# Huvinesh-Rajendran-12/keras-geometric

Measured on AMD Instinct MI355X. Metric: aggregated edges/sec + achieved HBM GB/s, GCNConv fwd, 1/2/4/8 MI355X, higher is better.
Workload: dtype fp32; 1 GPU; GCNConv fwd, R-MAT 10000000 nodes / 100000000 edges (+self loops), normalized, bias, F 128->128; nodes=10000000, edges=100000000, nodes_per_gpu=10000000, e_agg_per_gpu=110000000, max_in_degree=138539, mode=split-hub, fused aggregate->transform (W on bf16x3-split MFMA, f32-accurate), parallelism=single

## Files before the change

### include/kgx.h

```cpp
#ifndef KGX_H_
#define KGX_H_

#include <stddef.h>
#include <stdint.h>

#ifdef __cplusplus
extern "C" {
#endif

typedef void* kgx_stream_t;

enum kgx_status {
  KGX_OK = 0,
  KGX_ERR_ARG = 1,
  KGX_ERR_HIP = 2,
  KGX_ERR_INDEX = 3,
  KGX_ERR_UNSUPPORTED = 4
};

enum kgx_reduce { KGX_SUM = 0, KGX_MEAN = 1, KGX_MAX = 2, KGX_MIN = 3, KGX_STD = 4 };

enum kgx_epilogue { KGX_EPI_NONE = 0, KGX_EPI_BIAS = 1, KGX_EPI_GIN = 2, KGX_EPI_RAW = 3, KGX_EPI_ACCUM = 4 };

enum kgx_csr_flags {
  KGX_CSR_SELF_LOOPS = 1,
  KGX_CSR_SEGMENT_ONLY = 2,
  KGX_CSR_GCN_NORM = 4
};

int kgx_version(void);
const char* kgx_last_error(void);

int kgx_cu_split_layout_ok(int cus, int xccs, const char* arch);
int kgx_cu_split_supported(int device);
int kgx_cu_split_census(int per32, int64_t n_blocks, int32_t* head_ids, int32_t* tail_ids, int* n_cus,
                        kgx_stream_t stream);

int kgx_csr_workspace_bytes(int64_t E, int64_t n_dst, int flags, size_t* bytes);
int kgx_csr_build(const int32_t* src, const int32_t* dst, int64_t E,
                  int64_t n_src, int64_t n_dst, int flags,
                  int32_t* rowptr, int32_t* col, int32_t* eid, int32_t* deg,
                  float* dinv, float* w,
                  void* workspace, size_t workspace_bytes,
                  int64_t* info, kgx_stream_t stream);
int kgx_csr_build2(const int32_t* src, const int32_t* dst, int64_t E,
                   int64_t n_src, int64_t n_dst, int flags,
                   int32_t* rowptr, int32_t* col, int32_t* eid, int32_t* deg,
                   float* dinv, float* w, const float* dinv_table, int64_t table_len,
                   void* workspace, size_t workspace_bytes,
                   int64_t* info, kgx_stream_t stream);

int kgx_schedule_suffixes(const int32_t* items, int64_t n_items, int short_max, int tiny_max,
                          void* workspace, int64_t* out, kgx_stream_t stream);
int kgx_tiny_pack(const int32_t* items, int64_t start, int64_t n, const int32_t* col, const float* w,
                  int64_t n_col, int32_t* pack, float* tw, void* workspace, int64_t* out,
                  kgx_stream_t stream);

int kgx_gcn_dinv(const int32_t* deg, int64_t n, float* dinv, kgx_stream_t stream);
int kgx_gcn_dinv_table(const int32_t* deg, int64_t n, const float* table, int64_t table_len,
                       float* dinv, kgx_stream_t stream);
int kgx_gcn_edge_norm(const int32_t* rowptr, const int32_t* col, int64_t n_dst,
                      const float* dinv_dst, const float* dinv_src, float* w,
                      kgx_stream_t stream);

int kgx_schedule_workspace_bytes(int64_t n_dst, size_t* bytes);
int kgx_schedule_build(const int32_t* rowptr, int64_t n_dst, int32_t split_len,
                       int32_t* rows, int32_t* items, int64_t cap_items,
                       int32_t* split, void* workspace, size_t workspace_bytes,
                       int64_t* info, kgx_stream_t stream);

int kgx_spmm(int reduce, int epilogue,
             const int32_t* rowptr, const int32_t* rows, int64_t n_rows,
             const int32_t* items, int64_t n_items,
             const int32_t* split, int64_t n_split,
             const int32_t* idx, const float* w,
             const float* table, int64_t ld_table, int64_t F,
             float* out, int64_t ld_out,
             const float* bias, const float* xroot, int64_t ld_x, float gin_scale,
             const int32_t* drop_key, float drop_p, uint64_t drop_seed,
             float* partials, kgx_stream_t stream);
int kgx_spmm_ex(int reduce, int epilogue, const int32_t* rowptr, const int32_t* rows, int64_t n_rows,
                const int32_t* items, int64_t n_items, int64_t n_long_items, const int32_t* split,
                int64_t n_split, const int32_t* idx, const float* w, const float* table, int64_t ld_table,
                int64_t F, float* out, int64_t ld_out, const float* bias, const float* xroot, int64_t ld_x,
                float gin_scale, const int32_t* drop_key, float drop_p, uint64_t drop_seed, float* partials,
                kgx_stream_t stream);

int kgx_spmm_ex2(int reduce, int epilogue, const int32_t* rowptr, const int32_t* rows, int64_t n_rows,
                 const int32_t* items, int64_t n_items, int64_t n_long_items, const int32_t* split, int64_t n_split,
                 const int32_t* idx, const float* w, const float* table, int64_t ld_table, const float* table2,
                 int64_t n_table1, int64_t F, float* out, int64_t ld_out, const float* bias, const float* xroot,
                 int64_t ld_x, float gin_scale, const int32_t* drop_key, float drop_p, uint64_t drop_seed,
                 float* partials, int32_t* counters, kgx_stream_t stream);

int kgx_dropout_mask(uint64_t seed, float p, const int32_t* keys, int64_t n, int64_t F, float* out,
                     kgx_stream_t stream);

enum { KGX_FUSED_PRE_GIN = 1, KGX_FUSED_ACCUMULATE = 2, KGX_FUSED_SHARE_GPU = 4, KGX_FUSED_RELU = 8,
       KGX_FUSED_CU_SPLIT = 16 };
int kgx_spmm_gemm(int reduce, const int32_t* rowptr, const int32_t* rows, int64_t n_rows,
                  const int32_t* items, int64_t n_items, const int32_t* split, int64_t n_split,
                  const int32_t* idx, const float* w, const float* x, int64_t ld_x, int64_t F_in,
                  const float* W, int64_t F_out, const float* bias, int flags, float gin_scale,
                  float* out, int64_t ld_out, float* partials, float* agg_out, int64_t ld_agg,
                  kgx_stream_t stream);
enum { KGX_SHORT_ROW_MAX = 7 };
int kgx_spmm_gemm_ex(int reduce, const int32_t* rowptr, const int32_t* rows, int64_t n_rows,
                     const int32_t* items, int64_t n_items, int64_t n_long_items, const int32_t* split,
                     int64_t n_split, const int32_t* idx, const float* w, const float* x, int64_t ld_x,
                     int64_t F_in, const float* W, int64_t F_out, const float* bias, int flags,
                     float gin_scale, float* out, int64_t ld_out, float* partials, float* agg_out,
                     int64_t ld_agg, kgx_stream_t stream);

int kgx_spmm_gemm_ex2(int reduce, const int32_t* rowptr, const int32_t* rows, int64_t n_rows,
                      const int32_t* items, int64_t n_items, int64_t n_long_items, int64_t n_short_end,
                      const int32_t* tiny_pack, const float* tiny_w, int64_t n_tiny_deg2,
                      const int32_t* split, int64_t n_split,
                      const int32_t* idx, const float* w, const float* x, int64_t ld_x, int64_t F_in,
                      const float* W, int64_t F_out, const float* bias, int flags, float gin_scale, float* out,
                      int64_t ld_out, float* partials, float* agg_out, int64_t ld_agg, kgx_stream_t stream);

int kgx_spmm_gemm_ex3(int reduce, const int32_t* rowptr, const int32_t* rows, int64_t n_rows,
                      const int32_t* items, int64_t n_items, int64_t n_long_items, int64_t n_short_end,
                      const int32_t* tiny_pack, const float* tiny_w, int64_t n_tiny_deg2,
                      const int32_t* split, int64_t n_split, const int32_t* idx, const float* w,
                      const float* x, int64_t ld_x, const float* x2, int64_t n_x1, int64_t F_in,
                      const float* W, int64_t F_out, const float* bias, int flags, float gin_scale, float* out,
                      int64_t ld_out, float* partials, float* agg_out, int64_t ld_agg, kgx_stream_t stream);

int kgx_spmm_gemm_f256(int reduce, const int32_t* rowptr, const int32_t* rows, int64_t n_rows,
                       const int32_t* items, int64_t n_items, int64_t n_long_items, int64_t n_short_end,
                       const int32_t* tiny_pack, const float* tiny_w, const int32_t* split, int64_t n_split,
                       const int32_t* idx, const float* w, const float* x, int64_t ld_x, int64_t F_in,
                       const float* W, int64_t F_out, const float* bias, int flags, float gin_scale,
                       float* out, int64_t ld_out, float* partials, float* agg_out, int64_t ld_agg,
                       kgx_stream_t stream);

int kgx_spmm_gemm_f256_ex(int reduce, const int32_t* rowptr, const int32_t* rows, int64_t n_rows,
                          const int32_t* items, int64_t n_items, int64_t n_long_items, int64_t n_short_end,
                          const int32_t* tiny_pack, const float* tiny_w, const int32_t* split, int64_t n_split,
                          const int32_t* idx, const float* w, const float* x, int64_t ld_x, const float* x2,
                          int64_t n_x1, int64_t F_in, const float* W, int64_t F_out, const float* bias, int flags,
                          float gin_scale, float* out, int64_t ld_out, float* partials, float* agg_out,
                          int64_t ld_agg, kgx_stream_t stream);

int kgx_gemm_tn_workspace_bytes(int64_t N, int64_t K, int64_t M, size_t* bytes);
int kgx_gemm_tn(int64_t N, const float* P, int64_t ldp, int64_t K, const float* D, int64_t ldd, int64_t M,
                float* dW, int64_t ld_dw, float* db, void* workspace, size_t workspace_bytes,
                kgx_stream_t stream);

int kgx_spmm_max_backward(int reduce, int raw, const int32_t* rowptr, int64_t n_rows, const int32_t* idx,
                          const float* table, int64_t ld_table, int64_t F,
                          const float* grad_out, int64_t ld_grad_out,
                          float* grad_table, int64_t ld_grad_table, kgx_stream_t stream);

int kgx_gatv2(const int32_t* rowptr, const int32_t* rows, int64_t n_rows,
              const int32_t* items, int64_t n_items,
              const int32_t* split, int64_t n_split,
              const int32_t* col, const float* h_src, const float* h_dst, int64_t ld_h,
              const float* att, int heads, int channels, float negative_slope,
              float* out, int64_t ld_out, const float* bias,
              float* partials, float* stats,
              const int32_t* drop_key, float drop_p, uint64_t drop_seed, kgx_stream_t stream);

int kgx_gatv2_backward(const int32_t* rowptr, const int32_t* rows, int64_t n_rows,
                       const int32_t* items, int64_t n_items, const int32_t* split, int64_t n_split,
                       const int32_t* col, const float* h_src, const float* h_dst, int64_t ld_h,
                       const float* att, int heads, int channels, float negative_slope,
                       const float* out, int64_t ld_out, const float* bias, const float* stats,
                       const float* grad_out, int64_t ld_grad,
                       const int32_t* t_rowptr, const int32_t* t_rows, int64_t n_src,
                       const int32_t* t_items, int64_t t_n_items, const int32_t* t_split, int64_t t_n_split,
                       const int32_t* t_col, const int32_t* t_slot,
                       float* grad_h_src, float* grad_h_dst, int64_t ld_grad_h, float* grad_att,
                       float* alpha_ws, float* ds_ws, float* partials,
                       const int32_t* drop_key, float drop_p, uint64_t drop_seed, kgx_stream_t stream);

enum { KGX_POOL_SCORE_TANH = 1 };
enum { KGX_POOL_MAX_F = 256 };
int kgx_softmax_pool(const int32_t* rowptr, const int32_t* rows, int64_t n_seg,
                     const int32_t* items, int64_t n_items, const int32_t* split, int64_t n_split,
                     const int32_t* idx, const float* x, int64_t ld_x, int64_t F,
                     const float* s, const float* score_u, const float* score_c, int flags, float* s_out,
                     float* out, int64_t ld_out, float* stats, float* partials, kgx_stream_t stream);

int kgx_softmax_pool_backward(int64_t N, int64_t n_seg, const int32_t* seg,
                              const float* x, int64_t ld_x, int64_t F,
                              const float* s, const float* stats, const float* out, int64_t ld_out,
                              const float* grad_out, int64_t ld_grad,
                              float* grad_x, int64_t ld_grad_x, float* grad_s, kgx_stream_t stream);

enum { KGX_DENSE_RELU = 1, KGX_DENSE_ACCUMULATE = 2 };
enum { KGX_DENSE_MAX_K = 256, KGX_DENSE_MAX_N = 256 };
int kgx_dense(int64_t M, const float* x0, int64_t ld_x0, int64_t K0, const float* W0,
              const float* x1, int64_t ld_x1, int64_t K1, const float* W1, int64_t N,
              const float* bias, int flags, float* out, int64_t ld_out, kgx_stream_t stream);

int kgx_gather_rows(const float* table, int64_t ld_table, const int32_t* rows,
                    int64_t n, int64_t F, float* out, int64_t ld_out,
                    kgx_stream_t stream);
int kgx_scatter_f32(const float* in, const int32_t* perm, int64_t n, float* out,
                    kgx_stream_t stream);

int kgx_rmat_edges(uint64_t seed, int scale, int64_t n_nodes,
                   uint32_t a24, uint32_t b24, uint32_t c24,
                   int64_t e_begin, int64_t e_count,
                   int32_t* src, int32_t* dst, kgx_stream_t stream);

int kgx_select_dst_range(const int32_t* src, const int32_t* dst, int64_t n,
                         int64_t lo, int64_t hi, int32_t* src_out, int32_t* dst_out,
                         void* workspace, size_t workspace_bytes, int64_t* n_out,
                         kgx_stream_t stream);
int kgx_select_workspace_bytes(int64_t n, size_t* bytes);

int kgx_sample_workspace_bytes(int64_t n_seeds, size_t* bytes);
int kgx_sample_neighbors(const int32_t* rowptr, const int32_t* col, const int32_t* eid, int64_t n_rows,
                         const int32_t* seeds, int64_t n_seeds, int fanout, uint64_t seed, int hop,
                         int32_t* out_rowptr, int32_t* out_src, int32_t* out_eid, int64_t cap,
                         void* workspace, size_t workspace_bytes, int64_t* info, kgx_stream_t stream);
int kgx_relabel_workspace_bytes(int64_t n_edges, int64_t n_nodes, size_t* bytes);
int kgx_relabel_frontier(const int32_t* nodes, int64_t n_known, const int32_t* frontier, int64_t n_f,
                         const int32_t* out_rowptr, const int32_t* out_src, int64_t n_edges,
                         int32_t* map, int64_t n_nodes, int32_t* new_nodes, int32_t* src_local,
                         int32_t* dst_local, void* workspace, size_t workspace_bytes, int64_t* info,
                         kgx_stream_t stream);

#ifdef __cplusplus
}
#endif
#endif
```

### keras-geometric_amd/csrc/graph_build.hip

```cpp
#include <rocprim/device/device_radix_sort.hpp>
#include <rocprim/device/device_scan.hpp>

#include "kgx_internal.h"
#include "kgx_vec.h"

namespace kgx {
namespace {

struct CsrStatus {
  unsigned long long bad;
  unsigned long long max_deg;
  unsigned long long kept;
  unsigned long long table_miss;
};

__global__ void csr_prep_kernel(const int32_t* __restrict__ src, const int32_t* __restrict__ dst,
                                int64_t E, int64_t n_src, int64_t n_dst, int flags,
                                uint32_t* __restrict__ keys, uint64_t* __restrict__ vals,
                                CsrStatus* __restrict__ st) {
  const bool segment_only = flags & KGX_CSR_SEGMENT_ONLY;
  const bool loops = flags & KGX_CSR_SELF_LOOPS;
  const int64_t total = E + (loops ? n_dst : 0);
  const int64_t stride = int64_t(gridDim.x) * blockDim.x;
  unsigned long long bad = 0;
  for (int64_t e = int64_t(blockIdx.x) * blockDim.x + threadIdx.x; e < total; e += stride) {
    if (e < E) {
      int64_t s = src[e];
      int64_t d = dst[e];
      bool keep;
      if (segment_only) {
        keep = (d >= 0) && (d < n_dst);
      } else {
        const bool bad_e = (s < -n_src) || (s >= n_src) || (d < -n_dst) || (d >= n_dst);
        bad += bad_e;
        keep = !bad_e && d >= 0;
        if (s < 0) s += n_src;
      }
      keys[e] = keep ? uint32_t(d) : uint32_t(n_dst);
      vals[e] = (uint64_t(uint32_t(s)) << 32) | uint32_t(e);
    } else {
      const int64_t i = e - E;
      keys[e] = uint32_t(i);
      vals[e] = (uint64_t(uint32_t(i)) << 32) | uint32_t(e);
    }
  }
  if (bad) atomicAdd(&st->bad, bad);
}

__global__ void csr_rowptr_kernel(const uint32_t* __restrict__ keys, int64_t total, int64_t n_dst,
                                  int32_t* __restrict__ rowptr, CsrStatus* __restrict__ st) {
  const int64_t stride = int64_t(gridDim.x) * blockDim.x;
  for (int64_t r = int64_t(blockIdx.x) * blockDim.x + threadIdx.x; r <= n_dst; r += stride) {
    int64_t lo = 0, hi = total;
    const uint32_t key = uint32_t(r);
    while (lo < hi) {
      const int64_t mid = (lo + hi) >> 1;
      if (keys[mid] < key) lo = mid + 1; else hi = mid;
    }
    rowptr[r] = int32_t(lo);
    if (r == n_dst) st->kept = (unsigned long long)lo;
  }
}

constexpr int kColIlp = 4;

template <bool NORM>
__global__ void csr_col_kernel(const uint64_t* __restrict__ vals_sorted, const uint32_t* __restrict__ keys_sorted,
                               const int32_t* __restrict__ rowptr, int64_t n_dst, const float* __restrict__ dinv,
                               int32_t* __restrict__ eid, int32_t* __restrict__ col, float* __restrict__ w) {
  const int64_t kept = rowptr[n_dst];
  if (kept <= 0) return;
  const int64_t chunk = int64_t(blockDim.x) * kColIlp;
  for (int64_t base = int64_t(blockIdx.x) * chunk; base < kept; base += int64_t(gridDim.x) * chunk) {
    uint64_t v[kColIlp];
#pragma unroll
    for (int j = 0; j < kColIlp; ++j) {
      const int64_t e = base + int64_t(j) * blockDim.x + threadIdx.x;
      v[j] = vals_sorted[e < kept ? e : kept - 1];
    }
    if constexpr (NORM) {
      float dd[kColIlp], ds[kColIlp];
#pragma unroll
      for (int j = 0; j < kColIlp; ++j) {
        const int64_t e = base + int64_t(j) * blockDim.x + threadIdx.x;
        dd[j] = dinv[keys_sorted[e < kept ? e : kept - 1]];
        ds[j] = dinv[int32_t(v[j] >> 32)];
      }
#pragma unroll
      for (int j = 0; j < kColIlp; ++j) {
        const int64_t e = base + int64_t(j) * blockDim.x + threadIdx.x;
        if (e < kept) w[e] = __fmul_rn(dd[j], ds[j]);
      }
    }
#pragma unroll
    for (int j = 0; j < kColIlp; ++j) {
      const int64_t e = base + int64_t(j) * blockDim.x + threadIdx.x;
      if (e < kept) {
        eid[e] = int32_t(uint32_t(v[j]));
        col[e] = int32_t(v[j] >> 32);
      }
    }
  }
}


__device__ __forceinline__ float gcn_dinv(int32_t d) {
  return __fdiv_rn(1.0f, sqrt_rn(__fadd_rn(ref_count_f32(d), 1e-12f)));
}

__device__ __forceinline__ float gcn_dinv_lookup(int32_t d, const float* __restrict__ table, int64_t len,
                                                 unsigned* miss) {
  const int64_t k = d < (1 << 24) ? d : (1 << 24);
  if (k < len) return table[k];
  *miss += 1;
  return gcn_dinv(d);
}

__global__ void csr_deg_kernel(const int32_t* __restrict__ rowptr, int64_t n_dst, int flags,
                               int32_t* __restrict__ deg, float* __restrict__ dinv,
                               const float* __restrict__ table, int64_t table_len,
                               CsrStatus* __restrict__ st) {
  const int64_t stride = int64_t(gridDim.x) * blockDim.x;
  unsigned long long mx = 0;
  unsigned miss = 0;
  for (int64_t r = int64_t(blockIdx.x) * blockDim.x + threadIdx.x; r < n_dst; r += stride) {
    const int32_t d = rowptr[r + 1] - rowptr[r];
    deg[r] = d;
    mx = d > (int64_t)mx ? (unsigned long long)d : mx;
    if (flags & KGX_CSR_GCN_NORM) dinv[r] = table ? gcn_dinv_lookup(d, table, table_len, &miss) : gcn_dinv(d);
  }
  for (int o = 32; o > 0; o >>= 1) {
    unsigned long long other = __shfl_xor(mx, o, 64);
    mx = other > mx ? other : mx;
    miss += __shfl_xor(miss, o, 64);
  }
  __shared__ unsigned long long red_mx[kBlock / 64];
  __shared__ unsigned red_miss[kBlock / 64];
  if ((threadIdx.x & 63) == 0) {
    red_mx[threadIdx.x >> 6] = mx;
    red_miss[threadIdx.x >> 6] = miss;
  }
  __syncthreads();
  if (threadIdx.x == 0) {
    for (int k = 1; k < kBlock / 64; ++k) {
      mx = red_mx[k] > mx ? red_mx[k] : mx;
      miss += red_miss[k];
    }
    if (mx) atomicMax(&st->max_deg, mx);
    if (miss) atomicAdd(&st->table_miss, (unsigned long long)miss);
  }
}

size_t sort_temp_bytes(int64_t n, int end_bit) {
  size_t bytes = 0;
  uint32_t* k = nullptr;
  int32_t* v = nullptr;
  (void)rocprim::radix_sort_pairs(nullptr, bytes, k, k, v, v, (unsigned)n, 0, end_bit, 0, false);
  return bytes;
}

size_t sort_temp_bytes64(int64_t n, int end_bit) {
  size_t bytes = 0;
  uint32_t* k = nullptr;
  uint64_t* v = nullptr;
  (void)rocprim::radix_sort_pairs(nullptr, bytes, k, k, v, v, (unsigned)n, 0, end_bit, 0, false);
  return bytes;
}

struct CsrLayout {
  uint32_t* keys;
  uint32_t* keys_sorted;
  uint64_t* vals;
  uint64_t* vals_sorted;
  CsrStatus* st;
  void* sort_tmp;
  size_t sort_bytes;
  size_t total;
};

CsrLayout csr_layout(void* ws, int64_t total, int64_t n_dst) {
  Carve c(ws, ~size_t(0));
  CsrLayout L;
  L.keys = c.take<uint32_t>(total);
  L.keys_sorted = c.take<uint32_t>(total);
  L.vals = c.take<uint64_t>(total);
  L.vals_sorted = c.take<uint64_t>(total);
  L.st = c.take<CsrStatus>(1);
  const int end_bit = ceil_log2_u64(uint64_t(n_dst) + 1);
  L.sort_bytes = sort_temp_bytes64(total, end_bit > 0 ? end_bit : 1);
  L.sort_tmp = c.take<char>(L.sort_bytes);
  L.total = c.used();
  return L;
}

__global__ void gcn_dinv_kernel(const int32_t* __restrict__ deg, int64_t n, float* __restrict__ dinv) {
  const int64_t stride = int64_t(gridDim.x) * blockDim.x;
  for (int64_t i = int64_t(blockIdx.x) * blockDim.x + threadIdx.x; i < n; i += stride) dinv[i] = gcn_dinv(deg[i]);
}

__global__ void gcn_dinv_table_kernel(const int32_t* __restrict__ deg, int64_t n, const float* __restrict__ table,
                                      int64_t len, float* __restrict__ dinv) {
  const int64_t stride = int64_t(gridDim.x) * blockDim.x;
  for (int64_t i = int64_t(blockIdx.x) * blockDim.x + threadIdx.x; i < n; i += stride) {
    const int32_t d = deg[i];
    const int64_t k = d < (1 << 24) ? d : (1 << 24);
    dinv[i] = table[k < len ? k : len - 1];
  }
}

__global__ void gcn_edge_norm_kernel(const int32_t* __restrict__ rowptr, const int32_t* __restrict__ col,
                                     int64_t n_dst, const float* __restrict__ dinv_dst,
                                     const float* __restrict__ dinv_src, float* __restrict__ w) {
  const int sub = threadIdx.x & 7;
  const int64_t ng = (int64_t(gridDim.x) * blockDim.x) >> 3;
  for (int64_t r = (int64_t(blockIdx.x) * blockDim.x + threadIdx.x) >> 3; r < n_dst; r += ng) {
    const int32_t b = rowptr[r], e1 = rowptr[r + 1];
    if (e1 - b > 64) continue;
    const float dr = dinv_dst[r];
    for (int32_t e = b + sub; e < e1; e += 8) w[e] = __fmul_rn(dr, dinv_src[col[e]]);
  }
}

__global__ void gcn_edge_norm_long_kernel(const int32_t* __restrict__ rowptr, const int32_t* __restrict__ col,
                                          int64_t n_dst, const float* __restrict__ dinv_dst,
                                          const float* __restrict__ dinv_src, float* __restrict__ w) {
  const int lane = threadIdx.x & 63;
  const int64_t nw = (int64_t(gridDim.x) * blockDim.x) >> 6;
  for (int64_t r0 = ((int64_t(blockIdx.x) * blockDim.x + threadIdx.x) >> 6) * 64; r0 < n_dst; r0 += nw * 64) {
    const int64_t r = r0 + lane;
    const int32_t b = r < n_dst ? rowptr[r] : 0, e1 = r < n_dst ? rowptr[r + 1] : 0;
    unsigned long long long_rows = __ballot(e1 - b > 64);
    while (long_rows) {
      const int k = __ffsll(long_rows) - 1;
      long_rows &= long_rows - 1;
      const int32_t bk = __shfl(b, k, 64), ek = __shfl(e1, k, 64);
      const float dr = dinv_dst[r0 + k];
      for (int32_t e = bk + lane; e < ek; e += 64) w[e] = __fmul_rn(dr, dinv_src[col[e]]);
    }
  }
}

constexpr int kDegKeyBits = 24;
__device__ __forceinline__ uint32_t degree_key(int32_t d) {
  const uint32_t c = uint32_t(d) < (1u << kDegKeyBits) ? uint32_t(d) : (1u << kDegKeyBits) - 1u;
  return ((1u << kDegKeyBits) - 1u) - c;
}

__global__ void sched_keys_kernel(const int32_t* __restrict__ rowptr, int64_t n_dst,
                                  uint32_t* __restrict__ keys, int32_t* __restrict__ iota) {
  const int64_t stride = int64_t(gridDim.x) * blockDim.x;
  for (int64_t r = int64_t(blockIdx.x) * blockDim.x + threadIdx.x; r < n_dst; r += stride) {
    keys[r] = degree_key(rowptr[r + 1] - rowptr[r]);
    iota[r] = int32_t(r);
  }
}

__global__ void sched_count_kernel(const int32_t* __restrict__ rowptr, const int32_t* __restrict__ rows,
                                   int64_t n_dst, int32_t split_len, int32_t* __restrict__ nchunks,
                                   int32_t* __restrict__ nslots) {
  const int64_t stride = int64_t(gridDim.x) * blockDim.x;
  for (int64_t i = int64_t(blockIdx.x) * blockDim.x + threadIdx.x; i < n_dst; i += stride) {
    const int32_t r = rows[i];
    const int32_t d = rowptr[r + 1] - rowptr[r];
    const bool split = split_len > 0 && d >= split_len;
    const int32_t nc = split ? (d + split_len - 1) / split_len : 1;
    nchunks[i] = nc;
    nslots[i] = split ? nc : 0;
  }
}

struct SchedStatus {
  unsigned long long n_items;
  unsigned long long n_split;
  unsigned long long n_slots;
  unsigned long long overflow;
};

__global__ void sched_emit_kernel(const int32_t* __restrict__ rowptr, const int32_t* __restrict__ rows,
                                  int64_t n_dst, int32_t split_len,
                                  const int32_t* __restrict__ nchunks, const int32_t* __restrict__ item_off,
                                  const int32_t* __restrict__ nslots, const int32_t* __restrict__ slot_off,
                                  int4* __restrict__ items, int64_t cap_items, int4* __restrict__ split,
                                  SchedStatus* __restrict__ st) {
  const int64_t stride = int64_t(gridDim.x) * blockDim.x;
  unsigned long long nsplit = 0;
  for (int64_t i = int64_t(blockIdx.x) * blockDim.x + threadIdx.x; i < n_dst; i += stride) {
    const int32_t r = rows[i];
    const int32_t beg = rowptr[r];
    const int32_t end = rowptr[r + 1];
    const int32_t nc = nchunks[i];
    const int32_t off = item_off[i];
    if (int64_t(off) + nc > cap_items) {
      atomicAdd(&st->overflow, 1ull);
      continue;
    }
    if (nslots[i] > 0) {
      const int32_t s0 = slot_off[i];
      for (int32_t c = 0; c < nc; ++c) {
        const int32_t b = beg + c * split_len;
        const int32_t e = min(end, b + split_len);
        items[off + c] = make_int4(r, b, e, s0 + c);
      }
      split[i] = make_int4(r, s0, nc, end - beg);
      ++nsplit;
    } else {
      items[off] = make_int4(r, beg, end, -1);
    }
    if (i == n_dst - 1) {
      st->n_items = (unsigned long long)(off + nc);
      st->n_slots = (unsigned long long)(slot_off[i] + nslots[i]);
    }
  }
  if (nsplit) atomicAdd(&st->n_split, nsplit);
}

struct SchedLayout {
  uint32_t* keys;
  uint32_t* keys_sorted;
  int32_t* iota;
  int32_t* nchunks;
  int32_t* item_off;
  int32_t* nslots;
  int32_t* slot_off;
  SchedStatus* st;
  void* tmp;
  size_t tmp_bytes;
  size_t total;
};

SchedLayout sched_layout(void* ws, int64_t n) {
  Carve c(ws, ~size_t(0));
  SchedLayout L;
  L.keys = c.take<uint32_t>(n);
  L.keys_sorted = c.take<uint32_t>(n);
  L.iota = c.take<int32_t>(n);
  L.nchunks = c.take<int32_t>(n);
  L.item_off = c.take<int32_t>(n);
  L.nslots = c.take<int32_t>(n);
  L.slot_off = c.take<int32_t>(n);
  L.st = c.take<SchedStatus>(1);
  size_t sb = sort_temp_bytes(n, kDegKeyBits);
  size_t scb = 0;
  const int32_t* si = nullptr;
  int32_t* so = nullptr;
  (void)rocprim::exclusive_scan(nullptr, scb, si, so, 0, (size_t)n, rocprim::plus<int32_t>(), 0, false);
  L.tmp_bytes = sb > scb ? sb : scb;
  L.tmp = c.take<char>(L.tmp_bytes);
  L.total = c.used();
  return L;
}

__device__ __host__ __forceinline__ uint64_t splitmix64(uint64_t z) {
  z += 0x9E3779B97F4A7C15ull;
  z = (z ^ (z >> 30)) * 0xBF58476D1CE4E5B9ull;
  z = (z ^ (z >> 27)) * 0x94D049BB133111EBull;
  return z ^ (z >> 31);
}

struct Feistel {
  uint64_t keys[4];
  int hb;
  uint64_t mask;
};

__device__ __forceinline__ uint64_t feistel_once(const Feistel& f, uint64_t x) {
  uint64_t L = x >> f.hb, R = x & f.mask;
#pragma unroll
  for (int i = 0; i < 4; ++i) {
    const uint64_t nl = R;
    R = L ^ (splitmix64(f.keys[i] ^ R) & f.mask);
    L = nl;
  }
  return (L << f.hb) | R;
}

__device__ __forceinline__ uint64_t relabel(const Feistel& f, uint64_t x, uint64_t n) {
  uint64_t y = feistel_once(f, x);
  while (y >= n) y = feistel_once(f, y);
  return y;
}

__global__ void rmat_kernel(uint64_t base, Feistel fs, int scale, uint64_t n,
                            uint32_t ta, uint32_t tab, uint32_t tabc,
                            int64_t e_begin, int64_t e_count,
                            int32_t* __restrict__ src, int32_t* __restrict__ dst) {
  const int64_t stride = int64_t(gridDim.x) * blockDim.x;
  for (int64_t i = int64_t(blockIdx.x) * blockDim.x + threadIdx.x; i < e_count; i += stride) {
    const uint64_t k = uint64_t(e_begin + i);
    uint64_t s = 0, d = 0;
    for (int l = 0; l < scale; ++l) {
      const uint32_t r = uint32_t(splitmix64(base + k * 64ull + uint64_t(l)) >> 40);
      const uint32_t sb = r >= tab;
      const uint32_t db = (r >= ta && r < tab) || r >= tabc;
      s = (s << 1) | sb;
      d = (d << 1) | db;
    }
    src[i] = int32_t(relabel(fs, s % n, n));
    dst[i] = int32_t(relabel(fs, d % n, n));
  }
}

__global__ void range_flags_kernel(const int32_t* __restrict__ dst, int64_t n, int64_t lo, int64_t hi,
                                   int32_t* __restrict__ flags) {
  const int64_t stride = int64_t(gridDim.x) * blockDim.x;
  for (int64_t i = int64_t(blockIdx.x) * blockDim.x + threadIdx.x; i < n; i += stride) {
    const int64_t d = dst[i];
    flags[i] = (d >= lo && d < hi) ? 1 : 0;
  }
}

__global__ void range_scatter_kernel(const int32_t* __restrict__ src, const int32_t* __restrict__ dst,
                                     const int32_t* __restrict__ flags, const int32_t* __restrict__ pos,
                                     int64_t n, int32_t* __restrict__ so, int32_t* __restrict__ dout,
                                     unsigned long long* __restrict__ count) {
  const int64_t stride = int64_t(gridDim.x) * blockDim.x;
  for (int64_t i = int64_t(blockIdx.x) * blockDim.x + threadIdx.x; i < n; i += stride) {
    if (flags[i]) {
      so[pos[i]] = src[i];
      dout[pos[i]] = dst[i];
    }
    if (i == n - 1) *count = (unsigned long long)(pos[i] + flags[i]);
  }
}

template <int VEC>
__global__ void gather_rows_kernel(const float* __restrict__ table, int64_t ld_t,
                                   const int32_t* __restrict__ rows, int64_t n, int64_t F,
                                   float* __restrict__ out, int64_t ld_o) {
  using V = typename std::conditional<VEC == 4, float4, float>::type;
  const int64_t nv = F / VEC;
  const int64_t total = n * nv;
  const int64_t stride = int64_t(gridDim.x) * blockDim.x;
  for (int64_t t = int64_t(blockIdx.x) * blockDim.x + threadIdx.x; t < total; t += stride) {
    const int64_t i = t / nv, j = t - i * nv;
    const V v = *reinterpret_cast<const V*>(table + int64_t(rows[i]) * ld_t + j * VEC);
    *reinterpret_cast<V*>(out + i * ld_o + j * VEC) = v;
  }
}

__global__ void scatter_f32_kernel(const float* __restrict__ in, const int32_t* __restrict__ perm, int64_t n,
                                   float* __restrict__ out) {
  const int64_t stride = int64_t(gridDim.x) * blockDim.x;
  for (int64_t i = int64_t(blockIdx.x) * blockDim.x + threadIdx.x; i < n; i += stride)
    out[perm[i]] = in[i];
}

}
}

using namespace kgx;

extern "C" int kgx_csr_workspace_bytes(int64_t E, int64_t n_dst, int flags, size_t* bytes) {
  KGX_REQUIRE(bytes && E >= 0 && n_dst >= 0, KGX_ERR_ARG, "kgx_csr_workspace_bytes: bad arguments");
  const int64_t total = E + ((flags & KGX_CSR_SELF_LOOPS) ? n_dst : 0);
  *bytes = csr_layout(nullptr, total, n_dst).total;
  return KGX_OK;
}

extern "C" int kgx_csr_build2(const int32_t* src, const int32_t* dst, int64_t E, int64_t n_src,
                              int64_t n_dst, int flags, int32_t* rowptr, int32_t* col, int32_t* eid,
                              int32_t* deg, float* dinv, float* w, const float* dinv_table,
                              int64_t table_len, void* workspace, size_t workspace_bytes, int64_t* info,
                              kgx_stream_t stream_) {
  hipStream_t stream = as_stream(stream_);
  const bool loops = flags & KGX_CSR_SELF_LOOPS;
  const bool norm = flags & KGX_CSR_GCN_NORM;
  KGX_REQUIRE(E >= 0 && n_dst >= 0 && n_src >= 0, KGX_ERR_ARG, "kgx_csr_build: negative sizes");
  KGX_REQUIRE(!loops || n_src == n_dst, KGX_ERR_ARG,
              "kgx_csr_build: self loops need n_src == n_dst (got %lld, %lld)", (long long)n_src,
              (long long)n_dst);
  const int64_t total = E + (loops ? n_dst : 0);
  KGX_REQUIRE(total < (int64_t(1) << 31) - 1 && n_dst < (int64_t(1) << 31) - 1, KGX_ERR_ARG,
              "kgx_csr_build: graph too large for int32 CSR (E'=%lld)", (long long)total);
  KGX_REQUIRE(rowptr && deg && (total == 0 || (col && eid)), KGX_ERR_ARG, "kgx_csr_build: null output");
  KGX_REQUIRE(E == 0 || (src && dst), KGX_ERR_ARG, "kgx_csr_build: null input");
  KGX_REQUIRE(!norm || (dinv && (total == 0 || w)), KGX_ERR_ARG, "kgx_csr_build: GCN_NORM needs dinv and w");
  KGX_REQUIRE(!dinv_table || table_len > 0, KGX_ERR_ARG, "kgx_csr_build2: empty dinv table");
  CsrLayout L = csr_layout(workspace, total, n_dst);
  KGX_REQUIRE(workspace && workspace_bytes >= L.total, KGX_ERR_ARG,
              "kgx_csr_build: workspace %zu < %zu bytes", workspace_bytes, L.total);

  KGX_CHECK_HIP(hipMemsetAsync(L.st, 0, sizeof(CsrStatus), stream));
  if (total > 0) {
    hipLaunchKernelGGL(csr_prep_kernel, dim3(grid_for(total, 8192)), dim3(kBlock), 0, stream, src, dst, E,
                       n_src, n_dst, flags, L.keys, L.vals, L.st);
    KGX_CHECK_LAUNCH();
    const int end_bit = ceil_log2_u64(uint64_t(n_dst) + 1);
    size_t sb = L.sort_bytes;
    KGX_CHECK_HIP(rocprim::radix_sort_pairs(L.sort_tmp, sb, L.keys, L.keys_sorted, L.vals, L.vals_sorted,
                                            (unsigned)total, 0, end_bit > 0 ? end_bit : 1, stream,
                                            false));
  }
  hipLaunchKernelGGL(csr_rowptr_kernel, dim3(grid_for(n_dst + 1, 8192)), dim3(kBlock), 0, stream,
                     L.keys_sorted, total, n_dst, rowptr, L.st);
  KGX_CHECK_LAUNCH();
  if (n_dst > 0) {
    hipLaunchKernelGGL(csr_deg_kernel, dim3(grid_for(n_dst, 1024)), dim3(kBlock), 0, stream, rowptr, n_dst,
                       flags, deg, dinv, dinv_table, table_len, L.st);
    KGX_CHECK_LAUNCH();
  }
  if (total > 0) {
    const dim3 grid(grid_for(total / kColIlp + 1, 8192));
    if (norm)
      hipLaunchKernelGGL(csr_col_kernel<true>, grid, dim3(kBlock), 0, stream, L.vals_sorted, L.keys_sorted, rowptr,
                         n_dst, dinv, eid, col, w);
    else
      hipLaunchKernelGGL(csr_col_kernel<false>, grid, dim3(kBlock), 0, stream, L.vals_sorted, L.keys_sorted, rowptr,
                         n_dst, dinv, eid, col, w);
    KGX_CHECK_LAUNCH();
  }
  CsrStatus hs;
  KGX_CHECK_HIP(hipMemcpyAsync(&hs, L.st, sizeof(CsrStatus), hipMemcpyDeviceToHost, stream));
  KGX_CHECK_HIP(hipStreamSynchronize(stream));
  if (info) {
    info[0] = int64_t(hs.kept);
    info[1] = int64_t(hs.max_deg);
    info[2] = int64_t(hs.bad);
    info[3] = int64_t(hs.table_miss);
  }
  KGX_REQUIRE(hs.bad == 0, KGX_ERR_INDEX,
              "index out of range in edge_index: %llu edge(s) reference a node outside "
              "[-n, n) (n_src=%lld, n_dst=%lld)",
              hs.bad, (long long)n_src, (long long)n_dst);
  return KGX_OK;
}

extern "C" int kgx_csr_build(const int32_t* src, const int32_t* dst, int64_t E, int64_t n_src,
                             int64_t n_dst, int flags, int32_t* rowptr, int32_t* col, int32_t* eid,
                             int32_t* deg, float* dinv, float* w, void* workspace,
                             size_t workspace_bytes, int64_t* info, kgx_stream_t stream_) {
  return kgx_csr_build2(src, dst, E, n_src, n_dst, flags, rowptr, col, eid, deg, dinv, w, nullptr, 0, workspace,
                        workspace_bytes, info, stream_);
}

extern "C" int kgx_schedule_workspace_bytes(int64_t n_dst, size_t* bytes) {
  KGX_REQUIRE(bytes && n_dst >= 0, KGX_ERR_ARG, "kgx_schedule_workspace_bytes: bad arguments");
  *bytes = sched_layout(nullptr, n_dst).total;
  return KGX_OK;
}

extern "C" int kgx_schedule_build(const int32_t* rowptr, int64_t n_dst, int32_t split_len, int32_t* rows,
                                  int32_t* items, int64_t cap_items, int32_t* split, void* workspace,
                                  size_t workspace_bytes, int64_t* info, kgx_stream_t stream_) {
  hipStream_t stream = as_stream(stream_);
  KGX_REQUIRE(rowptr && n_dst >= 0, KGX_ERR_ARG, "kgx_schedule_build: bad arguments");
  KGX_REQUIRE(split_len <= 0 || (split_len & (split_len - 1)) == 0, KGX_ERR_ARG,
              "kgx_schedule_build: split_len must be a power of two (got %d)", split_len);
  if (n_dst == 0) {
    if (info) info[0] = info[1] = info[2] = info[3] = 0;
    return KGX_OK;
  }
  KGX_REQUIRE(rows && items && split, KGX_ERR_ARG, "kgx_schedule_build: null output");
  SchedLayout L = sched_layout(workspace, n_dst);
  KGX_REQUIRE(workspace && workspace_bytes >= L.total, KGX_ERR_ARG,
              "kgx_schedule_build: workspace %zu < %zu bytes", workspace_bytes, L.total);
  KGX_CHECK_HIP(hipMemsetAsync(L.st, 0, sizeof(SchedStatus), stream));
  const unsigned g = grid_for(n_dst, 8192);
  hipLaunchKernelGGL(sched_keys_kernel, dim3(g), dim3(kBlock), 0, stream, rowptr, n_dst, L.keys, L.iota);
  KGX_CHECK_LAUNCH();
  size_t tb = L.tmp_bytes;
  KGX_CHECK_HIP(rocprim::radix_sort_pairs(L.tmp, tb, L.keys, L.keys_sorted, L.iota, rows, (unsigned)n_dst, 0,
                                          kDegKeyBits, stream, false));
  hipLaunchKernelGGL(sched_count_kernel, dim3(g), dim3(kBlock), 0, stream, rowptr, rows, n_dst, split_len,
                     L.nchunks, L.nslots);
  KGX_CHECK_LAUNCH();
  tb = L.tmp_bytes;
  KGX_CHECK_HIP(rocprim::exclusive_scan(L.tmp, tb, (const int32_t*)L.nchunks, L.item_off, 0, (size_t)n_dst,
                                        rocprim::plus<int32_t>(), stream, false));
  tb = L.tmp_bytes;
  KGX_CHECK_HIP(rocprim::exclusive_scan(L.tmp, tb, (const int32_t*)L.nslots, L.slot_off, 0, (size_t)n_dst,
                                        rocprim::plus<int32_t>(), stream, false));
  hipLaunchKernelGGL(sched_emit_kernel, dim3(g), dim3(kBlock), 0, stream, rowptr, rows, n_dst, split_len,
                     L.nchunks, L.item_off, L.nslots, L.slot_off, reinterpret_cast<int4*>(items), cap_items,
                     reinterpret_cast<int4*>(split), L.st);
  KGX_CHECK_LAUNCH();
  SchedStatus hs;
  KGX_CHECK_HIP(hipMemcpyAsync(&hs, L.st, sizeof(SchedStatus), hipMemcpyDeviceToHost, stream));
  KGX_CHECK_HIP(hipStreamSynchronize(stream));
  KGX_REQUIRE(hs.overflow == 0, KGX_ERR_ARG, "kgx_schedule_build: cap_items %lld too small",
              (long long)cap_items);
  if (info) {
    info[0] = int64_t(hs.n_items);
    info[1] = int64_t(hs.n_split);
    info[2] = int64_t(hs.n_slots);
    info[3] = 0;
  }
  return KGX_OK;
}

extern "C" int kgx_rmat_edges(uint64_t seed, int scale, int64_t n_nodes, uint32_t a24, uint32_t b24,
                              uint32_t c24, int64_t e_begin, int64_t e_count, int32_t* src, int32_t* dst,
                              kgx_stream_t stream_) {
  hipStream_t stream = as_stream(stream_);
  KGX_REQUIRE(scale > 0 && scale <= 62 && n_nodes > 0 && n_nodes <= (int64_t(1) << scale) &&
                  n_nodes < (int64_t(1) << 31),
              KGX_ERR_ARG, "kgx_rmat_edges: need 0 < n_nodes <= 2^scale < 2^31 (scale=%d, n=%lld)", scale,
              (long long)n_nodes);
  KGX_REQUIRE(uint64_t(a24) + b24 + c24 <= (1u << 24), KGX_ERR_ARG, "kgx_rmat_edges: a+b+c > 1");
  KGX_REQUIRE(e_count >= 0 && e_begin >= 0 && (e_count == 0 || (src && dst)), KGX_ERR_ARG,
              "kgx_rmat_edges: bad edge range");
  if (e_count == 0) return KGX_OK;
  Feistel fs;
  fs.hb = (scale + 1) / 2;
  fs.mask = (uint64_t(1) << fs.hb) - 1;
  for (int i = 0; i < 4; ++i) fs.keys[i] = splitmix64(seed ^ (0xA5A5A5A5A5A5A5A5ull + uint64_t(i)));
  const uint64_t base = splitmix64(seed);
  hipLaunchKernelGGL(rmat_kernel, dim3(grid_for(e_count, 16384)), dim3(kBlock), 0, stream, base, fs, scale,
                     uint64_t(n_nodes), a24, a24 + b24, a24 + b24 + c24, e_begin, e_count, src, dst);
  KGX_CHECK_LAUNCH();
  return KGX_OK;
}

extern "C" int kgx_select_workspace_bytes(int64_t n, size_t* bytes) {
  KGX_REQUIRE(bytes && n >= 0, KGX_ERR_ARG, "kgx_select_workspace_bytes: bad arguments");
  size_t scb = 0;
  const int32_t* si = nullptr;
  int32_t* so = nullptr;
  (void)rocprim::exclusive_scan(nullptr, scb, si, so, 0, (size_t)(n > 0 ? n : 1), rocprim::plus<int32_t>(), 0,
                          false);
  Carve c(nullptr, ~size_t(0));
  c.take<int32_t>(n);
  c.take<int32_t>(n);
  c.take<unsigned long long>(1);
  c.take<char>(scb);
  *bytes = c.used();
  return KGX_OK;
}

extern "C" int kgx_select_dst_range(const int32_t* src, const int32_t* dst, int64_t n, int64_t lo, int64_t hi,
                                    int32_t* src_out, int32_t* dst_out, void* workspace, size_t workspace_bytes,
                                    int64_t* n_out, kgx_stream_t stream_) {
  hipStream_t stream = as_stream(stream_);
  KGX_REQUIRE(n >= 0 && n < (int64_t(1) << 31) && n_out, KGX_ERR_ARG, "kgx_select_dst_range: bad arguments");
  if (n == 0) {
    *n_out = 0;
    return KGX_OK;
  }
  size_t need = 0;
  kgx_select_workspace_bytes(n, &need);
  KGX_REQUIRE(workspace && workspace_bytes >= need, KGX_ERR_ARG, "kgx_select_dst_range: workspace too small");
  Carve c(workspace, workspace_bytes);
  int32_t* flags = c.take<int32_t>(n);
  int32_t* pos = c.take<int32_t>(n);
  unsigned long long* cnt = c.take<unsigned long long>(1);
  size_t scb = workspace_bytes - c.used();
  void* tmp = c.take<char>(0);
  const unsigned g = grid_for(n, 8192);
  hipLaunchKernelGGL(range_flags_kernel, dim3(g), dim3(kBlock), 0, stream, dst, n, lo, hi, flags);
  KGX_CHECK_LAUNCH();
  KGX_CHECK_HIP(rocprim::exclusive_scan(tmp, scb, (const int32_t*)flags, pos, 0, (size_t)n,
                                        rocprim::plus<int32_t>(), stream, false));
  hipLaunchKernelGGL(range_scatter_kernel, dim3(g), dim3(kBlock), 0, stream, src, dst, flags, pos, n, src_out,
                     dst_out, cnt);
  KGX_CHECK_LAUNCH();
  unsigned long long h = 0;
  KGX_CHECK_HIP(hipMemcpyAsync(&h, cnt, sizeof(h), hipMemcpyDeviceToHost, stream));
  KGX_CHECK_HIP(hipStreamSynchronize(stream));
  *n_out = int64_t(h);
  return KGX_OK;
}

extern "C" int kgx_gather_rows(const float* table, int64_t ld_table, const int32_t* rows, int64_t n, int64_t F,
                               float* out, int64_t ld_out, kgx_stream_t stream_) {
  hipStream_t stream = as_stream(stream_);
  KGX_REQUIRE(n >= 0 && F >= 0, KGX_ERR_ARG, "kgx_gather_rows: bad sizes");
  if (n == 0 || F == 0) return KGX_OK;
  KGX_REQUIRE(table && rows && out, KGX_ERR_ARG, "kgx_gather_rows: null pointer");
  const bool v4 = (F % 4 == 0) && (ld_table % 4 == 0) && (ld_out % 4 == 0) &&
                  (reinterpret_cast<uintptr_t>(table) % 16 == 0) && (reinterpret_cast<uintptr_t>(out) % 16 == 0);
  if (v4) {
    hipLaunchKernelGGL(gather_rows_kernel<4>, dim3(grid_for(n * (F / 4))), dim3(kBlock), 0, stream, table,
                       ld_table, rows, n, F, out, ld_out);
  } else {
    hipLaunchKernelGGL(gather_rows_kernel<1>, dim3(grid_for(n * F)), dim3(kBlock), 0, stream, table, ld_table,
                       rows, n, F, out, ld_out);
  }
  KGX_CHECK_LAUNCH();
  return KGX_OK;
}

extern "C" int kgx_scatter_f32(const float* in, const int32_t* perm, int64_t n, float* out,
                               kgx_stream_t stream_) {
  hipStream_t stream = as_stream(stream_);
  KGX_REQUIRE(n >= 0, KGX_ERR_ARG, "kgx_scatter_f32: bad size");
  if (n == 0) return KGX_OK;
  KGX_REQUIRE(in && perm && out, KGX_ERR_ARG, "kgx_scatter_f32: null pointer");
  hipLaunchKernelGGL(scatter_f32_kernel, dim3(grid_for(n)), dim3(kBlock), 0, stream, in, perm, n, out);
  KGX_CHECK_LAUNCH();
  return KGX_OK;
}

extern "C" int kgx_gcn_dinv(const int32_t* deg, int64_t n, float* dinv, kgx_stream_t stream_) {
  KGX_REQUIRE(n >= 0 && (n == 0 || (deg && dinv)), KGX_ERR_ARG, "kgx_gcn_dinv: bad arguments");
  if (n == 0) return KGX_OK;
  hipLaunchKernelGGL(gcn_dinv_kernel, dim3(grid_for(n, 8192)), dim3(kBlock), 0, as_stream(stream_), deg, n, dinv);
  KGX_CHECK_LAUNCH();
  return KGX_OK;
}

extern "C" int kgx_gcn_dinv_table(const int32_t* deg, int64_t n, const float* table, int64_t table_len, float* dinv,
                                  kgx_stream_t stream_) {
  KGX_REQUIRE(n >= 0 && (n == 0 || (deg && dinv && table && table_len > 0)), KGX_ERR_ARG,
              "kgx_gcn_dinv_table: bad arguments");
  if (n == 0) return KGX_OK;
  hipLaunchKernelGGL(gcn_dinv_table_kernel, dim3(grid_for(n, 8192)), dim3(kBlock), 0, as_stream(stream_), deg, n,
                     table, table_len, dinv);
  KGX_CHECK_LAUNCH();
  return KGX_OK;
}

extern "C" int kgx_gcn_edge_norm(const int32_t* rowptr, const int32_t* col, int64_t n_dst, const float* dinv_dst,
                                 const float* dinv_src, float* w, kgx_stream_t stream_) {
  KGX_REQUIRE(n_dst >= 0 && (n_dst == 0 || (rowptr && col && dinv_dst && dinv_src && w)), KGX_ERR_ARG,
              "kgx_gcn_edge_norm: bad arguments");
  if (n_dst == 0) return KGX_OK;
  hipStream_t s = as_stream(stream_);
  hipLaunchKernelGGL(gcn_edge_norm_kernel, dim3(grid_for(n_dst * 8, 8192)), dim3(kBlock), 0, s, rowptr, col, n_dst,
                     dinv_dst, dinv_src, w);
  KGX_CHECK_LAUNCH();
  hipLaunchKernelGGL(gcn_edge_norm_long_kernel, dim3(grid_for(n_dst, 8192)), dim3(kBlock), 0, s, rowptr, col,
                     n_dst, dinv_dst, dinv_src, w);
  KGX_CHECK_LAUNCH();
  return KGX_OK;
}

extern "C" int kgx_cu_split_layout_ok(int cus, int xccs, const char* arch) {
  return cu_split_layout_ok(cus, xccs, arch) ? 1 : 0;
}

extern "C" int kgx_cu_split_supported(int device) {
  int n = 0;
  KGX_CHECK_HIP(hipGetDeviceCount(&n));
  KGX_REQUIRE(device >= 0 && device < n, KGX_ERR_ARG, "kgx_cu_split_supported: no device %d", device);
  return cu_split_device_ok(device) ? 1 : 0;
}

namespace kgx {
namespace {
__global__ void cu_census_kernel(int32_t* __restrict__ ids, int64_t n) {
  unsigned hw, xcc;
  asm volatile("s_getreg_b32 %0, hwreg(HW_REG_HW_ID)" : "=s"(hw));
  asm volatile("s_getreg_b32 %0, hwreg(HW_REG_XCC_ID)" : "=s"(xcc));
  const int64_t t0 = wall_clock64();
  while (wall_clock64() - t0 < 2000) __builtin_amdgcn_s_sleep(8);
  if (threadIdx.x == 0 && int64_t(blockIdx.x) < n)
    ids[blockIdx.x] = int32_t(((xcc & 0xf) << 8) | (((hw >> 13) & 7) << 5) | (((hw >> 12) & 1) << 4) | ((hw >> 8) & 0xf));
}
}
}

extern "C" int kgx_cu_split_census(int per32, int64_t n_blocks, int32_t* head_ids, int32_t* tail_ids, int* n_cus,
                                   kgx_stream_t stream_) {
  KGX_REQUIRE(per32 > 0 && per32 < 32 && n_blocks > 0 && n_blocks <= (1 << 20) && head_ids && tail_ids && n_cus,
              KGX_ERR_ARG, "kgx_cu_split_census: bad arguments");
  hipStream_t s = as_stream(stream_);
  CuSplit* cs = cu_split(per32, s);
  KGX_REQUIRE(cs != nullptr, KGX_ERR_UNSUPPORTED, "kgx_cu_split_census: no CU split on this device / stream");
  SplitJoin sj;
  KGX_CHECK_HIP(sj.fork(cs, s));
  hipLaunchKernelGGL(cu_census_kernel, dim3(unsigned(n_blocks)), dim3(64), 0, cs->head, head_ids, n_blocks);
  KGX_CHECK_LAUNCH();
  hipLaunchKernelGGL(cu_census_kernel, dim3(unsigned(n_blocks)), dim3(64), 0, cs->tail, tail_ids, n_blocks);
  KGX_CHECK_LAUNCH();
  KGX_CHECK_HIP(sj.join());
  KGX_CHECK_HIP(hipStreamSynchronize(s));
  n_cus[0] = cs->n_head;
  n_cus[1] = cs->n_tail;
  return KGX_OK;
}

namespace kgx {
namespace {

__global__ void sched_suffix_kernel(const int4* __restrict__ items, int64_t n, int short_max, int tiny_max,
                                    unsigned long long* __restrict__ out) {
  const int64_t stride = int64_t(gridDim.x) * blockDim.x;
  unsigned long long ls = 0, lt = 0;
  for (int64_t i = int64_t(blockIdx.x) * blockDim.x + threadIdx.x; i < n; i += stride) {
    const int4 v = items[i];
    const int len = v.z - v.y;
    if (v.w >= 0 || len > short_max) ls = (unsigned long long)(i + 1);
    if (v.w >= 0 || len > tiny_max) lt = (unsigned long long)(i + 1);
  }
  for (int o = 32; o > 0; o >>= 1) {
    const unsigned long long a = __shfl_xor(ls, o, 64), b = __shfl_xor(lt, o, 64);
    ls = a > ls ? a : ls;
    lt = b > lt ? b : lt;
  }
  __shared__ unsigned long long red[2][kBlock / 64];
  const int wv = threadIdx.x >> 6;
  if ((threadIdx.x & 63) == 0) {
    red[0][wv] = ls;
    red[1][wv] = lt;
  }
  __syncthreads();
  if (threadIdx.x == 0) {
    for (int k = 1; k < kBlock / 64; ++k) {
      ls = red[0][k] > ls ? red[0][k] : ls;
      lt = red[1][k] > lt ? red[1][k] : lt;
    }
    if (ls) atomicMax(&out[0], ls);
    if (lt) atomicMax(&out[1], lt);
  }
}

__global__ void tiny_pack_kernel(const int4* __restrict__ items, int64_t start, int64_t n,
                                 const int32_t* __restrict__ col, const float* __restrict__ w, int64_t n_col,
                                 int4* __restrict__ pack, float2* __restrict__ tw, unsigned long long* __restrict__ st) {
  const int64_t stride = int64_t(gridDim.x) * blockDim.x;
  unsigned long long cnt = 0, last2 = 0;
  for (int64_t i = int64_t(blockIdx.x) * blockDim.x + threadIdx.x; i < n; i += stride) {
    const int4 v = items[start + i];
    const int deg = v.z - v.y;
    const int64_t last = n_col - 1;
    const int64_t i0 = v.y < last ? v.y : last;
    const int64_t i1b = int64_t(v.y) + (deg > 1 ? 1 : 0);
    const int64_t i1 = i1b < last ? i1b : last;
    const int32_t c0 = deg > 0 ? col[i0] : 0, c1 = deg > 0 ? col[i1] : 0;
    pack[i] = make_int4(v.x, deg, c0, c1);
    if (tw) tw[i] = make_float2(deg > 0 ? w[i0] : 0.0f, deg > 1 ? w[i1] : 0.0f);
    if (deg == 2) {
      ++cnt;
      last2 = (unsigned long long)(i + 1);
    }
  }
  for (int o = 32; o > 0; o >>= 1) {
    cnt += __shfl_xor(cnt, o, 64);
    const unsigned long long b = __shfl_xor(last2, o, 64);
    last2 = b > last2 ? b : last2;
  }
  __shared__ unsigned long long red[2][kBlock / 64];
  const int wv = threadIdx.x >> 6;
  if ((threadIdx.x & 63) == 0) {
    red[0][wv] = cnt;
    red[1][wv] = last2;
  }
  __syncthreads();
  if (threadIdx.x == 0) {
    for (int k = 1; k < kBlock / 64; ++k) {
      cnt += red[0][k];
      last2 = red[1][k] > last2 ? red[1][k] : last2;
    }
    if (cnt) atomicAdd(&st[0], cnt);
    if (last2) atomicMax(&st[1], last2);
  }
}

}
}

extern "C" int kgx_schedule_suffixes(const int32_t* items, int64_t n_items, int short_max, int tiny_max,
                                     void* workspace, int64_t* out, kgx_stream_t stream_) {
  KGX_REQUIRE(n_items >= 0 && out && workspace && (n_items == 0 || items), KGX_ERR_ARG,
              "kgx_schedule_suffixes: bad arguments");
  hipStream_t s = as_stream(stream_);
  auto* st = static_cast<unsigned long long*>(workspace);
  KGX_CHECK_HIP(hipMemsetAsync(st, 0, 2 * sizeof(unsigned long long), s));
  if (n_items > 0) {
    hipLaunchKernelGGL(sched_suffix_kernel, dim3(grid_for(n_items, 1024)), dim3(kBlock), 0, s,
                       reinterpret_cast<const int4*>(items), n_items, short_max, tiny_max, st);
    KGX_CHECK_LAUNCH();
  }
  unsigned long long h[2];
  KGX_CHECK_HIP(hipMemcpyAsync(h, st, sizeof(h), hipMemcpyDeviceToHost, s));
  KGX_CHECK_HIP(hipStreamSynchronize(s));
  out[0] = int64_t(h[0]);
  out[1] = int64_t(h[1]);
  return KGX_OK;
}

extern "C" int kgx_tiny_pack(const int32_t* items, int64_t start, int64_t n, const int32_t* col, const float* w,
                             int64_t n_col, int32_t* pack, float* tw, void* workspace, int64_t* out,
                             kgx_stream_t stream_) {
  KGX_REQUIRE(start >= 0 && n >= 0 && n_col > 0 && items && col && pack && workspace && out && (!tw || w),
              KGX_ERR_ARG, "kgx_tiny_pack: bad arguments");
  hipStream_t s = as_stream(stream_);
  auto* st = static_cast<unsigned long long*>(workspace);
  KGX_CHECK_HIP(hipMemsetAsync(st, 0, 2 * sizeof(unsigned long long), s));
  if (n > 0) {
    hipLaunchKernelGGL(tiny_pack_kernel, dim3(grid_for(n, 2048)), dim3(kBlock), 0, s,
                       reinterpret_cast<const int4*>(items), start, n, col, tw ? w : nullptr, n_col,
                       reinterpret_cast<int4*>(pack), reinterpret_cast<float2*>(tw), st);
    KGX_CHECK_LAUNCH();
  }
  unsigned long long h[2];
  KGX_CHECK_HIP(hipMemcpyAsync(h, st, sizeof(h), hipMemcpyDeviceToHost, s));
  KGX_CHECK_HIP(hipStreamSynchronize(s));
  out[0] = int64_t(h[0]);
  out[1] = int64_t(h[1]);
  return KGX_OK;
}
```

### keras-geometric_amd/keras_geometric_amd/_native.py

```python

from __future__ import annotations

import ctypes
import os
from pathlib import Path

import torch

_PKG_ROOT = Path(__file__).resolve().parent.parent
LIB_PATH = Path(os.environ.get("KGX_LIB", _PKG_ROOT / "lib" / "libkgx.so"))

KGX_OK, KGX_ERR_ARG, KGX_ERR_HIP, KGX_ERR_INDEX, KGX_ERR_UNSUPPORTED = range(5)
SUM, MEAN, MAX, MIN, STD = range(5)
EPI_NONE, EPI_BIAS, EPI_GIN, EPI_RAW, EPI_ACCUM = range(5)
FUSED_PRE_GIN, FUSED_ACCUMULATE, FUSED_SHARE_GPU, FUSED_RELU, FUSED_CU_SPLIT = 1, 2, 4, 8, 16
CSR_SELF_LOOPS, CSR_SEGMENT_ONLY, CSR_GCN_NORM = 1, 2, 4
DENSE_RELU, DENSE_ACCUMULATE = 1, 2
DENSE_MAX_K, DENSE_MAX_N = 256, 256
POOL_SCORE_TANH = 1
POOL_MAX_F = 256

REDUCE_IDS = {"sum": SUM, "mean": MEAN, "max": MAX, "min": MIN, "std": STD}

_i32p = ctypes.c_void_p
_f32p = ctypes.c_void_p
_i64 = ctypes.c_int64
_int = ctypes.c_int

_SIGNATURES = {
    "kgx_version": [],
    "kgx_last_error": [],
    "kgx_csr_workspace_bytes": [_i64, _i64, _int, ctypes.POINTER(ctypes.c_size_t)],
    "kgx_csr_build": [
        _i32p, _i32p, _i64, _i64, _i64, _int,
        _i32p, _i32p, _i32p, _i32p, _f32p, _f32p,
        ctypes.c_void_p, ctypes.c_size_t, ctypes.POINTER(ctypes.c_int64), ctypes.c_void_p,
    ],
    "kgx_csr_build2": [
        _i32p, _i32p, _i64, _i64, _i64, _int,
        _i32p, _i32p, _i32p, _i32p, _f32p, _f32p, _f32p, _i64,
        ctypes.c_void_p, ctypes.c_size_t, ctypes.POINTER(ctypes.c_int64), ctypes.c_void_p,
    ],
    "kgx_gcn_dinv": [_i32p, _i64, _f32p, ctypes.c_void_p],
    "kgx_cu_split_layout_ok": [_int, _int, ctypes.c_char_p],
    "kgx_schedule_suffixes": [_i32p, _i64, _int, _int, ctypes.c_void_p, ctypes.POINTER(ctypes.c_int64),
                              ctypes.c_void_p],
    "kgx_tiny_pack": [_i32p, _i64, _i64, _i32p, _f32p, _i64, _i32p, _f32p, ctypes.c_void_p,
                      ctypes.POINTER(ctypes.c_int64), ctypes.c_void_p],
    "kgx_gemm_tn_workspace_bytes": [_i64, _i64, _i64, ctypes.POINTER(ctypes.c_size_t)],
    "kgx_gemm_tn": [_i64, _f32p, _i64, _i64, _f32p, _i64, _i64, _f32p, _i64, _f32p, ctypes.c_void_p,
                    ctypes.c_size_t, ctypes.c_void_p],
    "kgx_cu_split_supported": [_int],
    "kgx_cu_split_census": [_int, _i64, _i32p, _i32p, ctypes.POINTER(ctypes.c_int), ctypes.c_void_p],
    "kgx_gcn_dinv_table": [_i32p, _i64, _f32p, _i64, _f32p, ctypes.c_void_p],
    "kgx_gcn_edge_norm": [_i32p, _i32p, _i64, _f32p, _f32p, _f32p, ctypes.c_void_p],
    "kgx_schedule_workspace_bytes": [_i64, ctypes.POINTER(ctypes.c_size_t)],
    "kgx_schedule_build": [
        _i32p, _i64, ctypes.c_int32, _i32p, _i32p, _i64, _i32p,
        ctypes.c_void_p, ctypes.c_size_t, ctypes.POINTER(ctypes.c_int64), ctypes.c_void_p,
    ],
    "kgx_spmm": [
        _int, _int, _i32p, _i32p, _i64, _i32p, _i64, _i32p, _i64,
        _i32p, _f32p, _f32p, _i64, _i64, _f32p, _i64,
        _f32p, _f32p, _i64, ctypes.c_float, _i32p, ctypes.c_float, ctypes.c_uint64, _f32p, ctypes.c_void_p,
    ],
    "kgx_spmm_ex": [
        _int, _int, _i32p, _i32p, _i64, _i32p, _i64, _i64, _i32p, _i64,
        _i32p, _f32p, _f32p, _i64, _i64, _f32p, _i64,
        _f32p, _f32p, _i64, ctypes.c_float, _i32p, ctypes.c_float, ctypes.c_uint64, _f32p, ctypes.c_void_p,
    ],
    "kgx_spmm_ex2": [
        _int, _int, _i32p, _i32p, _i64, _i32p, _i64, _i64, _i32p, _i64,
        _i32p, _f32p, _f32p, _i64, _f32p, _i64, _i64, _f32p, _i64,
        _f32p, _f32p, _i64, ctypes.c_float, _i32p, ctypes.c_float, ctypes.c_uint64, _f32p, _i32p, ctypes.c_void_p,
    ],
    "kgx_dropout_mask": [ctypes.c_uint64, ctypes.c_float, _i32p, _i64, _i64, _f32p, ctypes.c_void_p],
    "kgx_spmm_gemm": [
        _int, _i32p, _i32p, _i64, _i32p, _i64, _i32p, _i64,
        _i32p, _f32p, _f32p, _i64, _i64, _f32p, _i64, _f32p, _int, ctypes.c_float,
        _f32p, _i64, _f32p, _f32p, _i64, ctypes.c_void_p,
    ],
    "kgx_spmm_gemm_ex": [
        _int, _i32p, _i32p, _i64, _i32p, _i64, _i64, _i32p, _i64,
        _i32p, _f32p, _f32p, _i64, _i64, _f32p, _i64, _f32p, _int, ctypes.c_float,
        _f32p, _i64, _f32p, _f32p, _i64, ctypes.c_void_p,
    ],
    "kgx_spmm_gemm_ex2": [
        _int, _i32p, _i32p, _i64, _i32p, _i64, _i64, _i64, _i32p, _f32p, _i64, _i32p, _i64,
        _i32p, _f32p, _f32p, _i64, _i64, _f32p, _i64, _f32p, _int, ctypes.c_float,
        _f32p, _i64, _f32p, _f32p, _i64, ctypes.c_void_p,
    ],
    "kgx_spmm_gemm_f256": [
        _int, _i32p, _i32p, _i64, _i32p, _i64, _i64, _i64, _i32p, _f32p, _i32p, _i64,
        _i32p, _f32p, _f32p, _i64, _i64, _f32p, _i64, _f32p, _int, ctypes.c_float,
        _f32p, _i64, _f32p, _f32p, _i64, ctypes.c_void_p,
    ],
    "kgx_spmm_gemm_f256_ex": [
        _int, _i32p, _i32p, _i64, _i32p, _i64, _i64, _i64, _i32p, _f32p, _i32p, _i64,
        _i32p, _f32p, _f32p, _i64, _f32p, _i64, _i64, _f32p, _i64, _f32p, _int, ctypes.c_float,
        _f32p, _i64, _f32p, _f32p, _i64, ctypes.c_void_p,
    ],
    "kgx_spmm_gemm_ex3": [
        _int, _i32p, _i32p, _i64, _i32p, _i64, _i64, _i64, _i32p, _f32p, _i64, _i32p, _i64,
        _i32p, _f32p, _f32p, _i64, _f32p, _i64, _i64, _f32p, _i64, _f32p, _int, ctypes.c_float,
        _f32p, _i64, _f32p, _f32p, _i64, ctypes.c_void_p,
    ],
    "kgx_spmm_max_backward": [
        _int, _int, _i32p, _i64, _i32p, _f32p, _i64, _i64, _f32p, _i64, _f32p, _i64, ctypes.c_void_p,
    ],
    "kgx_gatv2_backward": [
        _i32p, _i32p, _i64, _i32p, _i64, _i32p, _i64, _i32p, _f32p, _f32p, _i64, _f32p, _int, _int,
        ctypes.c_float, _f32p, _i64, _f32p, _f32p, _f32p, _i64,
        _i32p, _i32p, _i64, _i32p, _i64, _i32p, _i64, _i32p, _i32p,
        _f32p, _f32p, _i64, _f32p, _f32p, _f32p, _f32p, _i32p, ctypes.c_float, ctypes.c_uint64, ctypes.c_void_p,
    ],
    "kgx_gatv2": [
        _i32p, _i32p, _i64, _i32p, _i64, _i32p, _i64,
        _i32p, _f32p, _f32p, _i64, _f32p, _int, _int, ctypes.c_float,
        _f32p, _i64, _f32p, _f32p, _f32p, _i32p, ctypes.c_float, ctypes.c_uint64, ctypes.c_void_p,
    ],
    "kgx_softmax_pool": [
        _i32p, _i32p, _i64, _i32p, _i64, _i32p, _i64, _i32p, _f32p, _i64, _i64,
        _f32p, _f32p, _f32p, _int, _f32p, _f32p, _i64, _f32p, _f32p, ctypes.c_void_p,
    ],
    "kgx_softmax_pool_backward": [
        _i64, _i64, _i32p, _f32p, _i64, _i64, _f32p, _f32p, _f32p, _i64, _f32p, _i64, _f32p, _i64, _f32p,
        ctypes.c_void_p,
    ],
    "kgx_dense": [
        _i64, _f32p, _i64, _i64, _f32p, _f32p, _i64, _i64, _f32p, _i64, _f32p, _int, _f32p, _i64, ctypes.c_void_p,
    ],
    "kgx_gather_rows": [_f32p, _i64, _i32p, _i64, _i64, _f32p, _i64, ctypes.c_void_p],
    "kgx_scatter_f32": [_f32p, _i32p, _i64, _f32p, ctypes.c_void_p],
    "kgx_rmat_edges": [
        ctypes.c_uint64, _int, _i64, ctypes.c_uint32, ctypes.c_uint32, ctypes.c_uint32,
        _i64, _i64, _i32p, _i32p, ctypes.c_void_p,
    ],
    "kgx_select_workspace_bytes": [_i64, ctypes.POINTER(ctypes.c_size_t)],
    "kgx_select_dst_range": [
        _i32p, _i32p, _i64, _i64, _i64, _i32p, _i32p,
        ctypes.c_void_p, ctypes.c_size_t, ctypes.POINTER(ctypes.c_int64), ctypes.c_void_p,
    ],
    "kgx_sample_workspace_bytes": [_i64, ctypes.POINTER(ctypes.c_size_t)],
    "kgx_sample_neighbors": [
        _i32p, _i32p, _i32p, _i64, _i32p, _i64, _int, ctypes.c_uint64, _int,
        _i32p, _i32p, _i32p, _i64,
        ctypes.c_void_p, ctypes.c_size_t, ctypes.POINTER(ctypes.c_int64), ctypes.c_void_p,
    ],
    "kgx_relabel_workspace_bytes": [_i64, _i64, ctypes.POINTER(ctypes.c_size_t)],
    "kgx_relabel_frontier": [
        _i32p, _i64, _i32p, _i64, _i32p, _i32p, _i64,
        _i32p, _i64, _i32p, _i32p, _i32p,
        ctypes.c_void_p, ctypes.c_size_t, ctypes.POINTER(ctypes.c_int64), ctypes.c_void_p,
    ],
}
_RESTYPES = {"kgx_last_error": ctypes.c_char_p}

_lib: ctypes.CDLL | None = None


def lib() -> ctypes.CDLL:
    global _lib
    if _lib is None:
        if not LIB_PATH.exists():
            raise RuntimeError(
                f"kgx native library not found at {LIB_PATH}. Build it with "
                "`make -C keras-geometric_amd/csrc` (or __graft_entry__.build())."
            )
        handle = ctypes.CDLL(str(LIB_PATH))
        for name, argtypes in _SIGNATURES.items():
            fn = getattr(handle, name)
            fn.argtypes = argtypes
            fn.restype = _RESTYPES.get(name, ctypes.c_int)
        _lib = handle
    return _lib


def exported_symbols() -> list[str]:
    return list(_SIGNATURES)


def check(rc: int, what: str) -> None:
    if rc == KGX_OK:
        return
    msg = lib().kgx_last_error().decode(errors="replace")
    if rc == KGX_ERR_INDEX:
        raise IndexError(msg)
    if rc in (KGX_ERR_ARG, KGX_ERR_UNSUPPORTED):
        raise ValueError(f"{what}: {msg}")
    raise RuntimeError(f"{what} failed (status {rc}): {msg}")


def require_device(*tensors: torch.Tensor | None) -> torch.device:
    dev = None
    for t in tensors:
        if t is None:
            continue
        if t.device.type != "cuda":
            raise RuntimeError(
                "kgx kernels run on MI355X (ROCm) only: got a tensor on "
                f"{t.device}. Move inputs to a cuda device; there is no CPU path."
            )
        if dev is None:
            dev = t.device
        elif t.device != dev:
            raise RuntimeError(f"kgx: tensors on different devices ({dev} vs {t.device})")
    if dev is None:
        raise RuntimeError("kgx: no device tensor given")
    return dev


def ptr(t: torch.Tensor | None) -> ctypes.c_void_p | None:
    return None if t is None else ctypes.c_void_p(t.data_ptr())


def stream(device: torch.device) -> ctypes.c_void_p:
    return ctypes.c_void_p(torch.cuda.current_stream(device).cuda_stream)
```

### keras-geometric_amd/keras_geometric_amd/graph.py

```python

from __future__ import annotations

import ctypes
import os
from collections import OrderedDict
from dataclasses import dataclass, field

import numpy as np
import torch

from . import _native as nat

_ASSUMED_GROUP_SLOTS = 2048 * 256


def _pow2_floor(v: int) -> int:
    return 1 << (max(int(v), 1).bit_length() - 1)


def default_split_len(n_edges: int, n_features: int = 128) -> int:
    lanes = max(1, (max(n_features, 1) + 3) // 4)
    G = min(64, 1 << (lanes - 1).bit_length())
    groups = _ASSUMED_GROUP_SLOTS // G
    share = max(1, n_edges // groups)
    return int(min(8192, max(256, _pow2_floor(max(share // 4, 1)))))


def exact_mode_default() -> bool:
    return os.environ.get("KGX_EXACT", "0") not in ("", "0", "false", "False")


@dataclass
class CSRGraph:
    n_src: int
    n_dst: int
    n_input_edges: int
    kept: int
    max_degree: int
    flags: int
    rowptr: torch.Tensor
    col: torch.Tensor
    eid: torch.Tensor
    deg: torch.Tensor
    dinv: torch.Tensor | None = None
    w: torch.Tensor | None = None
    rows: torch.Tensor | None = None
    items: torch.Tensor | None = None
    split: torch.Tensor | None = None
    n_items: int = 0
    n_split: int = 0
    n_slots: int = 0
    split_len: int = 0
    n_long: int = -1
    extras: dict = field(default_factory=dict)

    @property
    def device(self) -> torch.device:
        return self.rowptr.device

    def work(self, exact: bool):
        if exact or self.n_items == 0:
            return None, 0, None, 0, 0
        return self.items, self.n_items, self.split, self.n_split, self.n_slots


_DINV_TABLES: dict = {}
_DINV_SLICE = 16384


def _dinv_values(lo: int, hi: int) -> torch.Tensor:
    out = []
    exp = torch.tensor(-0.5, dtype=torch.float32)
    for a in range(lo - lo % _DINV_SLICE, hi, _DINV_SLICE):
        k = torch.arange(a, a + _DINV_SLICE, dtype=torch.float32)
        out.append(torch.pow(torch.add(k, torch.tensor(1e-12, dtype=torch.float32)), exp))
    vals = torch.cat(out)
    off = lo - (lo - lo % _DINV_SLICE)
    return vals[off: off + hi - lo]


def gcn_dinv_table(device: torch.device, max_degree: int = 0) -> torch.Tensor:
    need = min(max(int(max_degree), 0), 1 << 24) + 1
    key = str(torch.device(device))
    t = _DINV_TABLES.get(key)
    if t is None or t.numel() < need:
        n = max(4096, 1 << (need - 1).bit_length())
        n = min(n, (1 << 24) + 1)
        t = _dinv_values(0, n).to(device)
        _DINV_TABLES[key] = t
    return t


def build_csr(
    src: torch.Tensor,
    dst: torch.Tensor,
    n_src: int,
    n_dst: int,
    *,
    self_loops: bool = False,
    gcn_norm: bool = False,
    segment_only: bool = False,
    split_len: int | None = None,
    n_features: int = 128,
) -> CSRGraph:
    dev = nat.require_device(src, dst)
    if src.dtype != torch.int32 or dst.dtype != torch.int32:
        raise TypeError("build_csr expects int32 src/dst")
    src = src.contiguous()
    dst = dst.contiguous()
    E = int(src.numel())
    if int(dst.numel()) != E:
        raise ValueError(f"src/dst length mismatch: {E} vs {dst.numel()}")
    flags = (
        (nat.CSR_SELF_LOOPS if self_loops else 0)
        | (nat.CSR_SEGMENT_ONLY if segment_only else 0)
        | (nat.CSR_GCN_NORM if gcn_norm else 0)
    )
    cap = E + (n_dst if self_loops else 0)
    L = nat.lib()
    i32 = dict(dtype=torch.int32, device=dev)
    rowptr = torch.empty(n_dst + 1, **i32)
    col = torch.empty(max(cap, 1), **i32)
    eid = torch.empty(max(cap, 1), **i32)
    deg = torch.empty(max(n_dst, 1), **i32)
    dinv = torch.empty(max(n_dst, 1), dtype=torch.float32, device=dev) if gcn_norm else None
    w = torch.empty(max(cap, 1), dtype=torch.float32, device=dev) if gcn_norm else None
    nbytes = ctypes.c_size_t(0)
    nat.check(L.kgx_csr_workspace_bytes(E, n_dst, flags, ctypes.byref(nbytes)), "kgx_csr_workspace_bytes")
    ws = torch.empty(max(nbytes.value, 1), dtype=torch.uint8, device=dev)
    info = (ctypes.c_int64 * 4)()
    table = gcn_dinv_table(dev) if gcn_norm else None
    nat.check(
        L.kgx_csr_build2(
            nat.ptr(src), nat.ptr(dst), E, n_src, n_dst, flags,
            nat.ptr(rowptr), nat.ptr(col), nat.ptr(eid), nat.ptr(deg), nat.ptr(dinv), nat.ptr(w),
            nat.ptr(table), table.numel() if table is not None else 0,
            nat.ptr(ws), nbytes.value, info, nat.stream(dev),
        ),
        "kgx_csr_build2",
    )
    del ws
    kept, max_deg = int(info[0]), int(info[1])
    if gcn_norm and int(info[3]):
        table = gcn_dinv_table(dev, max_deg)
        st = nat.stream(dev)
        nat.check(L.kgx_gcn_dinv_table(nat.ptr(deg), n_dst, nat.ptr(table), table.numel(), nat.ptr(dinv), st),
                  "kgx_gcn_dinv_table")
        nat.check(L.kgx_gcn_edge_norm(nat.ptr(rowptr), nat.ptr(col), n_dst, nat.ptr(dinv), nat.ptr(dinv),
                                      nat.ptr(w), st), "kgx_gcn_edge_norm")
    g = CSRGraph(
        n_src=n_src, n_dst=n_dst, n_input_edges=E, kept=kept, max_degree=max_deg, flags=flags,
        rowptr=rowptr, col=col[:kept], eid=eid[:kept], deg=deg[:n_dst],
        dinv=dinv[:n_dst] if dinv is not None else None, w=w[:kept] if w is not None else None,
    )
    _build_schedule(g, split_len if split_len is not None else default_split_len(kept, n_features))
    return g


def _build_schedule(g: CSRGraph, split_len: int, tails: bool = True) -> None:
    dev = g.device
    n = g.n_dst
    if split_len > 0:
        split_len = _pow2_floor(split_len)
    g.split_len = split_len
    if n == 0:
        g.rows = torch.empty(0, dtype=torch.int32, device=dev)
        return
    L = nat.lib()
    cap_items = n + (g.kept // split_len if split_len > 0 else 0) + 1
    cap_split = min(n, (g.kept // split_len if split_len > 0 else 0) + 1)
    rows = torch.empty(n, dtype=torch.int32, device=dev)
    items = torch.empty((cap_items, 4), dtype=torch.int32, device=dev)
    split = torch.empty((max(cap_split, 1), 4), dtype=torch.int32, device=dev)
    nbytes = ctypes.c_size_t(0)
    nat.check(L.kgx_schedule_workspace_bytes(n, ctypes.byref(nbytes)), "kgx_schedule_workspace_bytes")
    ws = torch.empty(max(nbytes.value, 1), dtype=torch.uint8, device=dev)
    info = (ctypes.c_int64 * 4)()
    nat.check(
        L.kgx_schedule_build(
            nat.ptr(g.rowptr), n, split_len, nat.ptr(rows), nat.ptr(items), cap_items, nat.ptr(split),
            nat.ptr(ws), nbytes.value, info, nat.stream(dev),
        ),
        "kgx_schedule_build",
    )
    g.rows = rows
    g.n_items, g.n_split, g.n_slots = int(info[0]), int(info[1]), int(info[2])
    if g.n_split > cap_split:
        raise RuntimeError("kgx schedule: split list overflow")
    g.items = items[: g.n_items]
    g.split = split[: max(g.n_split, 0)]
    if not tails:
        return
    g.n_long = short_suffix_start(g.items)
    _refresh_tiny(g)


POOL_CHUNK_MAX = 1024
_POOL_TARGET_ITEMS = 2048


def pool_chunk_len(n_nodes: int) -> int:
    env = os.environ.get("KGX_POOL_CHUNK")
    if env:
        return _pow2_floor(int(env))
    return int(min(POOL_CHUNK_MAX, max(64, _pow2_floor(max(n_nodes // _POOL_TARGET_ITEMS, 1)))))


_SINGLE_SEGMENTS: "OrderedDict[tuple, CSRGraph]" = OrderedDict()


def single_segment_graph(n_nodes: int, device: torch.device, chunk_len: int | None = None) -> CSRGraph:
    chunk = pool_chunk_len(n_nodes) if chunk_len is None else int(chunk_len)
    key = (int(n_nodes), str(torch.device(device)), chunk)
    g = _SINGLE_SEGMENTS.get(key)
    if g is None:
        dev = torch.device(device)
        g = CSRGraph(
            n_src=n_nodes, n_dst=1, n_input_edges=n_nodes, kept=n_nodes, max_degree=n_nodes, flags=nat.CSR_SEGMENT_ONLY,
            rowptr=torch.tensor([0, n_nodes], dtype=torch.int32, device=dev), col=None, eid=None,
            deg=torch.tensor([n_nodes], dtype=torch.int32, device=dev),
        )
        _build_schedule(g, chunk, tails=False)
        _SINGLE_SEGMENTS[key] = g
        while len(_SINGLE_SEGMENTS) > 16:
            _SINGLE_SEGMENTS.popitem(last=False)
    return g


def segment_of_node(g: CSRGraph) -> torch.Tensor | None:
    if g.col is None:
        return None
    seg = g.extras.get("segment_of_node")
    if seg is None:
        seg = torch.full((g.n_src,), -1, dtype=torch.int32, device=g.device)
        if g.kept:
            seg[g.col.long()] = row_of_slot(g)
        g.extras["segment_of_node"] = seg
    return seg


def _refresh_tiny(g: CSRGraph) -> None:
    from . import tiny

    tiny.tiny_pack(g, refresh=True)


SHORT_ROW_MAX = 7


def schedule_suffixes(items: torch.Tensor, short_max: int, tiny_max: int) -> tuple[int, int]:
    n = int(items.shape[0])
    if n == 0:
        return 0, 0
    ws = torch.empty(16, dtype=torch.uint8, device=items.device)
    out = (ctypes.c_int64 * 2)()
    nat.check(nat.lib().kgx_schedule_suffixes(nat.ptr(items.contiguous()), n, int(short_max), int(tiny_max),
                                              nat.ptr(ws), out, nat.stream(items.device)), "kgx_schedule_suffixes")
    return int(out[0]), int(out[1])


def short_suffix_start(items: torch.Tensor) -> int:
    n = int(items.shape[0])
    if n == 0 or os.environ.get("KGX_SHORT_ROWS", "1") in ("0", "false", "False"):
        return n
    smax = int(os.environ.get("KGX_SHORT_MAX", SHORT_ROW_MAX))
    if items.is_cuda:
        return schedule_suffixes(items, smax, smax)[0]
    short = ((items[:, 2] - items[:, 1]) <= smax) & (items[:, 3] < 0)
    not_short = torch.nonzero(~short)
    return int(not_short[-1]) + 1 if not_short.numel() else 0


def exact_short_start(g: CSRGraph) -> int:
    hit = g.extras.get("exact_short")
    if hit is not None:
        return hit
    n = -1
    if g.rows is not None and g.n_dst > 0 and os.environ.get("KGX_SHORT_ROWS", "1") not in ("0", "false", "False"):
        smax = int(os.environ.get("KGX_SHORT_MAX", SHORT_ROW_MAX))
        k = int((g.deg[g.rows.long()] > smax).sum())
        n = k if 0 < k < g.n_dst else -1
    g.extras["exact_short"] = n
    return n


def row_of_slot(g: CSRGraph) -> torch.Tensor:
    r = g.extras.get("row_of_slot")
    if r is None:
        if g.kept:
            r = torch.repeat_interleave(torch.arange(g.n_dst, device=g.device, dtype=torch.int32),
                                        g.deg.long(), output_size=g.kept)
        else:
            r = torch.empty(0, dtype=torch.int32, device=g.device)
        g.extras["row_of_slot"] = r
    return r


def transpose(g: CSRGraph) -> CSRGraph:
    t = g.extras.get("T")
    if t is not None:
        return t
    if g.kept:
        order = torch.sort(g.eid, stable=True).indices
        src_t = row_of_slot(g)[order].contiguous()
        dst_t = g.col[order].contiguous()
    else:
        order = torch.empty(0, dtype=torch.int64, device=g.device)
        src_t = dst_t = torch.empty(0, dtype=torch.int32, device=g.device)
    t = build_csr(src_t, dst_t, g.n_dst, g.n_src)
    slot = order[t.eid.long()] if t.kept else order
    t.eid = g.eid[slot].contiguous() if t.kept else g.eid[:0]
    if g.w is not None:
        t.w = g.w[slot].contiguous()
        _refresh_tiny(t)
    t.extras["fwd_slot"] = slot
    g.extras["T"] = t
    return t


def split_by_source(g: CSRGraph, n_own: int) -> tuple[CSRGraph, CSRGraph]:
    own, other = split_by_source_ranges(g, [0, n_own, g.n_src], accumulate_from=2)
    return own, other


def split_by_source_ranges(g: CSRGraph, cuts: list[int], accumulate_from: int = 1) -> list[CSRGraph]:
    if len(cuts) < 2 or cuts[0] != 0 or cuts[-1] != g.n_src or any(a > b for a, b in zip(cuts, cuts[1:])):
        raise ValueError(f"split_by_source_ranges: cuts must rise from 0 to n_src={g.n_src} (got {cuts})")
    part_of = torch.bucketize(g.col, torch.tensor(cuts[1:-1], dtype=torch.int32, device=g.device), right=True)
    return split_by_part(g, part_of, [(cuts[k], cuts[k + 1] - cuts[k]) for k in range(len(cuts) - 1)],
                         accumulate_from)


def split_by_part(g: CSRGraph, part_of: torch.Tensor, sources: list, accumulate_from: int = 1) -> list[CSRGraph]:
    row_of = row_of_slot(g)
    parts = []
    for k, (base, n_src) in enumerate(sources):
        m = part_of == k
        deg = torch.bincount(row_of[m], minlength=g.n_dst).to(torch.int32)[: g.n_dst]
        rowptr = torch.zeros(g.n_dst + 1, dtype=torch.int32, device=g.device)
        rowptr[1:] = torch.cumsum(deg, 0)
        col = g.col[m] - base if base else g.col[m]
        kept = int(col.numel())
        sub = CSRGraph(
            n_src=n_src, n_dst=g.n_dst, n_input_edges=kept, kept=kept,
            max_degree=int(deg.max()) if g.n_dst else 0, flags=g.flags,
            rowptr=rowptr, col=col.contiguous(), eid=g.eid[m].contiguous(), deg=deg,
            dinv=g.dinv, w=g.w[m].contiguous() if g.w is not None else None,
        )
        _build_schedule(sub, default_split_len(kept))
        if k >= accumulate_from and sub.n_items:
            empty = int((deg == 0).sum())
            sub.n_items -= empty
            sub.items = sub.items[: sub.n_items]
            sub.n_long = min(sub.n_long, sub.n_items)
            sub.extras["accumulate_only"] = True
            _refresh_tiny(sub)
        parts.append(sub)
    return parts


def restrict_rows(g: CSRGraph, row_mask: torch.Tensor) -> CSRGraph:
    from dataclasses import replace

    if g.n_items == 0:
        return replace(g, extras={})
    keep = row_mask[g.items[:, 0].long()]
    items = g.items[keep].contiguous()
    split = g.split[row_mask[g.split[:, 0].long()]].contiguous() if g.n_split else g.split
    sub = replace(g, items=items, split=split, n_items=int(items.shape[0]), n_split=int(split.shape[0]) if g.n_split
                  else 0, extras={"restricted_of": g})
    sub.n_long = short_suffix_start(items)
    _refresh_tiny(sub)
    return sub


_CACHE: "OrderedDict[tuple, tuple[torch.Tensor, CSRGraph]]" = OrderedDict()
_CACHE_SIZE = int(os.environ.get("KGX_GRAPH_CACHE", "8"))


def host_array_key(a) -> tuple | None:
    if not isinstance(a, np.ndarray):
        return None
    n = a.size
    pick = np.linspace(0, n - 1, min(n, 4096)).astype(np.int64) if n else np.zeros(0, np.int64)
    sample = np.ascontiguousarray(a.flat[pick])
    return ("host", id(a), a.__array_interface__["data"][0], a.shape, a.strides, a.dtype.str,
            hash(sample.tobytes()))


def cache_key(edge_index: torch.Tensor, *extra) -> tuple | None:
    if not isinstance(edge_index, torch.Tensor):
        hk = host_array_key(edge_index)
        return (*hk, *extra) if hk is not None else None
    return (
        edge_index.data_ptr(), edge_index._version, tuple(edge_index.shape), tuple(edge_index.stride()),
        edge_index.dtype, str(edge_index.device), *extra,
    )


def cached(key: tuple | None, anchor, builder) -> CSRGraph:
    if key is None or _CACHE_SIZE <= 0:
        return builder()
    hit = _CACHE.get(key)
    if hit is not None:
        _CACHE.move_to_end(key)
        return hit[1]
    g = builder()
    _CACHE[key] = (anchor, g)
    while len(_CACHE) > _CACHE_SIZE:
        _CACHE.popitem(last=False)
    return g


def clear_cache() -> None:
    _CACHE.clear()
    from .layers import _edges

    _edges._HOST_CAST.clear()
```

Measured before the change: 12.85 billion edges/s.

## Fuse CSR build and schedule into one native call with lazy edge ids

Graph construction now sorts packed 64-bit (dst,src) keys instead of key/value pairs with edge ids, places self loops analytically rather than sorting them, and defers building the eid array until it is first read. The CSR build, schedule and tiny-row packing are merged into one native call so fewer host round-trips and stream syncs occur. This targets graph-build cost and does not touch the aggregation kernel. If the metric covers only the forward pass with a cached graph, little effect is expected. The lazy eid path adds a risk of stale data if the source edge index is modified in place.

```diff
diff --git a/include/kgx.h b/include/kgx.h
--- a/include/kgx.h
+++ b/include/kgx.h
@@ -49,6 +49,20 @@
                    float* dinv, float* w, const float* dinv_table, int64_t table_len,
                    void* workspace, size_t workspace_bytes,
                    int64_t* info, kgx_stream_t stream);
+
+int kgx_csr_workspace_bytes2(int64_t E, int64_t n_dst, int flags, int with_eid, size_t* bytes);
+int kgx_csr_eid_workspace_bytes(int64_t E, int64_t n_dst, size_t* bytes);
+int kgx_csr_eid(const int32_t* dst, int64_t E, int64_t n_dst, int flags, const int32_t* rowptr,
+                int32_t* eid, void* workspace, size_t workspace_bytes, kgx_stream_t stream);
+
+int kgx_graph_build_workspace_bytes(int64_t E, int64_t n_dst, int flags, size_t* bytes);
+int kgx_graph_build(const int32_t* src, const int32_t* dst, int64_t E, int64_t n_src, int64_t n_dst,
+                    int flags, int32_t* rowptr, int32_t* col, int32_t* deg, float* dinv, float* w,
+                    const float* dinv_table, int64_t table_len, int32_t split_len, int32_t* rows,
+                    int32_t* items, int64_t cap_items, int32_t* split, int short_max, int tiny_max,
+                    int64_t tiny_min_rows, int32_t* pack, float* tw, int64_t tiny_cap,
+                    void* workspace, size_t workspace_bytes, int64_t* info, kgx_stream_t stream);
+int64_t kgx_graph_sync_count(void);
 
 int kgx_schedule_suffixes(const int32_t* items, int64_t n_items, int short_max, int tiny_max,
                           void* workspace, int64_t* out, kgx_stream_t stream);
diff --git a/keras-geometric_amd/csrc/graph_build.hip b/keras-geometric_amd/csrc/graph_build.hip
--- a/keras-geometric_amd/csrc/graph_build.hip
+++ b/keras-geometric_amd/csrc/graph_build.hip
@@ -1,11 +1,19 @@
 #include <rocprim/device/device_radix_sort.hpp>
 #include <rocprim/device/device_scan.hpp>
 
+#include <atomic>
+
 #include "kgx_internal.h"
 #include "kgx_vec.h"
 
 namespace kgx {
 namespace {
+
+std::atomic<long long> g_stream_syncs{0};
+inline hipError_t sync_counted(hipStream_t s) {
+  g_stream_syncs.fetch_add(1, std::memory_order_relaxed);
+  return hipStreamSynchronize(s);
+}
 
 struct CsrStatus {
   unsigned long long bad;
@@ -47,7 +55,8 @@
   if (bad) atomicAdd(&st->bad, bad);
 }
 
-__global__ void csr_rowptr_kernel(const uint32_t* __restrict__ keys, int64_t total, int64_t n_dst,
+template <typename K, int SHIFT>
+__global__ void csr_rowptr_kernel(const K* __restrict__ keys, int64_t total, int64_t n_dst, int loops_apart,
                                   int32_t* __restrict__ rowptr, CsrStatus* __restrict__ st) {
   const int64_t stride = int64_t(gridDim.x) * blockDim.x;
   for (int64_t r = int64_t(blockIdx.x) * blockDim.x + threadIdx.x; r <= n_dst; r += stride) {
@@ -55,11 +64,35 @@
     const uint32_t key = uint32_t(r);
     while (lo < hi) {
       const int64_t mid = (lo + hi) >> 1;
-      if (keys[mid] < key) lo = mid + 1; else hi = mid;
-    }
+      if (uint32_t(keys[mid] >> SHIFT) < key) lo = mid + 1; else hi = mid;
+    }
+    if (loops_apart) lo += r;
     rowptr[r] = int32_t(lo);
     if (r == n_dst) st->kept = (unsigned long long)lo;
   }
+}
+
+__global__ void csr_prep64_kernel(const int32_t* __restrict__ src, const int32_t* __restrict__ dst,
+                                  int64_t E, int64_t n_src, int64_t n_dst, int flags,
+                                  uint64_t* __restrict__ keys, CsrStatus* __restrict__ st) {
+  const bool segment_only = flags & KGX_CSR_SEGMENT_ONLY;
+  const int64_t stride = int64_t(gridDim.x) * blockDim.x;
+  unsigned long long bad = 0;
+  for (int64_t e = int64_t(blockIdx.x) * blockDim.x + threadIdx.x; e < E; e += stride) {
+    int64_t s = src[e];
+    const int64_t d = dst[e];
+    bool keep;
+    if (segment_only) {
+      keep = (d >= 0) && (d < n_dst);
+    } else {
+      const bool bad_e = (s < -n_src) || (s >= n_src) || (d < -n_dst) || (d >= n_dst);
+      bad += bad_e;
+      keep = !bad_e && d >= 0;
+      if (s < 0) s += n_src;
+    }
+    keys[e] = (uint64_t(keep ? uint32_t(d) : uint32_t(n_dst)) << 32) | uint32_t(s);
+  }
+  if (bad) atomicAdd(&st->bad, bad);
 }
 
 constexpr int kColIlp = 4;
@@ -103,6 +136,71 @@
   }
 }
 
+template <bool NORM>
+__global__ void csr_col64_kernel(const uint64_t* __restrict__ keys_sorted, const int32_t* __restrict__ rowptr,
+                                 int64_t n_dst, int loops_apart, const float* __restrict__ dinv,
+                                 int32_t* __restrict__ col, float* __restrict__ w) {
+  const int64_t kept = int64_t(rowptr[n_dst]) - (loops_apart ? n_dst : 0);
+  if (kept <= 0) return;
+  const int64_t chunk = int64_t(blockDim.x) * kColIlp;
+  for (int64_t base = int64_t(blockIdx.x) * chunk; base < kept; base += int64_t(gridDim.x) * chunk) {
+    uint64_t v[kColIlp];
+#pragma unroll
+    for (int j = 0; j < kColIlp; ++j) {
+      const int64_t e = base + int64_t(j) * blockDim.x + threadIdx.x;
+      v[j] = keys_sorted[e < kept ? e : kept - 1];
+    }
+    float dd[kColIlp], ds[kColIlp];
+    if constexpr (NORM) {
+#pragma unroll
+      for (int j = 0; j < kColIlp; ++j) {
+        dd[j] = dinv[uint32_t(v[j] >> 32)];
+        ds[j] = dinv[int32_t(uint32_t(v[j]))];
+      }
+    }
+#pragma unroll
+    for (int j = 0; j < kColIlp; ++j) {
+      const int64_t e = base + int64_t(j) * blockDim.x + threadIdx.x;
+      if (e < kept) {
+        const int64_t slot = e + (loops_apart ? int64_t(v[j] >> 32) : 0);
+        col[slot] = int32_t(uint32_t(v[j]));
+        if constexpr (NORM) w[slot] = __fmul_rn(dd[j], ds[j]);
+      }
+    }
+  }
+}
+
+__global__ void eid_prep_kernel(const int32_t* __restrict__ dst, int64_t E, int64_t n_dst,
+                                uint32_t* __restrict__ keys, uint32_t* __restrict__ vals) {
+  const int64_t stride = int64_t(gridDim.x) * blockDim.x;
+  for (int64_t e = int64_t(blockIdx.x) * blockDim.x + threadIdx.x; e < E; e += stride) {
+    const int64_t d = dst[e];
+    keys[e] = (d >= 0 && d < n_dst) ? uint32_t(d) : uint32_t(n_dst);
+    vals[e] = uint32_t(e);
+  }
+}
+
+__global__ void eid_place_kernel(const uint32_t* __restrict__ keys_sorted, const uint32_t* __restrict__ vals_sorted,
+                                 const int32_t* __restrict__ rowptr, int64_t E, int64_t n_dst, int loops,
+                                 int32_t* __restrict__ eid) {
+  const int64_t kept_all = rowptr[n_dst];
+  const int64_t kept_in = kept_all - (loops ? n_dst : 0);
+  const int64_t kept = kept_in < E ? kept_in : E;
+  const int64_t stride = int64_t(gridDim.x) * blockDim.x;
+  const int64_t t0 = int64_t(blockIdx.x) * blockDim.x + threadIdx.x;
+  for (int64_t p = t0; p < kept; p += stride) {
+    const uint32_t d = keys_sorted[p];
+    if (int64_t(d) >= n_dst) continue;
+    eid[p + (loops ? int64_t(d) : 0)] = int32_t(vals_sorted[p]);
+  }
+  if (loops) {
+    for (int64_t r = t0; r < n_dst; r += stride) {
+      const int64_t slot = int64_t(rowptr[r + 1]) - 1;
+      if (slot >= 0 && slot < E + n_dst) eid[slot] = int32_t(E + r);
+    }
+  }
+}
+
 
 __device__ __forceinline__ float gcn_dinv(int32_t d) {
   return __fdiv_rn(1.0f, sqrt_rn(__fadd_rn(ref_count_f32(d), 1e-12f)));
@@ -119,15 +217,25 @@
 __global__ void csr_deg_kernel(const int32_t* __restrict__ rowptr, int64_t n_dst, int flags,
                                int32_t* __restrict__ deg, float* __restrict__ dinv,
                                const float* __restrict__ table, int64_t table_len,
-                               CsrStatus* __restrict__ st) {
+                               CsrStatus* __restrict__ st, int32_t* __restrict__ loop_col,
+                               float* __restrict__ loop_w) {
   const int64_t stride = int64_t(gridDim.x) * blockDim.x;
   unsigned long long mx = 0;
   unsigned miss = 0;
   for (int64_t r = int64_t(blockIdx.x) * blockDim.x + threadIdx.x; r < n_dst; r += stride) {
-    const int32_t d = rowptr[r + 1] - rowptr[r];
+    const int32_t end = rowptr[r + 1];
+    const int32_t d = end - rowptr[r];
     deg[r] = d;
     mx = d > (int64_t)mx ? (unsigned long long)d : mx;
-    if (flags & KGX_CSR_GCN_NORM) dinv[r] = table ? gcn_dinv_lookup(d, table, table_len, &miss) : gcn_dinv(d);
+    float di = 0.0f;
+    if (flags & KGX_CSR_GCN_NORM) {
+      di = table ? gcn_dinv_lookup(d, table, table_len, &miss) : gcn_dinv(d);
+      dinv[r] = di;
+    }
+    if (loop_col) {
+      loop_col[end - 1] = int32_t(r);
+      if (flags & KGX_CSR_GCN_NORM) loop_w[end - 1] = __fmul_rn(di, di);
+    }
   }
   for (int o = 32; o > 0; o >>= 1) {
     unsigned long long other = __shfl_xor(mx, o, 64);
@@ -188,6 +296,64 @@
   L.st = c.take<CsrStatus>(1);
   const int end_bit = ceil_log2_u64(uint64_t(n_dst) + 1);
   L.sort_bytes = sort_temp_bytes64(total, end_bit > 0 ? end_bit : 1);
+  L.sort_tmp = c.take<char>(L.sort_bytes);
+  L.total = c.used();
+  return L;
+}
+
+size_t sort_temp_bytes_keys64(int64_t n, int end_bit) {
+  size_t bytes = 0;
+  rocprim::double_buffer<uint64_t> k(nullptr, nullptr);
+  (void)rocprim::radix_sort_keys(nullptr, bytes, k, (unsigned)n, 32, 32 + end_bit, 0, false);
+  return bytes;
+}
+
+struct Csr64Layout {
+  uint64_t* keys;
+  uint64_t* keys_alt;
+  CsrStatus* st;
+  void* sort_tmp;
+  size_t sort_bytes;
+  size_t total;
+};
+
+inline int csr_end_bit(int64_t n_dst) {
+  const int b = ceil_log2_u64(uint64_t(n_dst) + 1);
+  return b > 0 ? b : 1;
+}
+
+Csr64Layout csr64_layout(void* ws, int64_t E, int64_t n_dst) {
+  Carve c(ws, ~size_t(0));
+  Csr64Layout L;
+  L.st = c.take<CsrStatus>(1);
+  L.keys = c.take<uint64_t>(E);
+  L.keys_alt = c.take<uint64_t>(E);
+  L.sort_bytes = sort_temp_bytes_keys64(E, csr_end_bit(n_dst));
+  L.sort_tmp = c.take<char>(L.sort_bytes);
+  L.total = c.used();
+  return L;
+}
+
+struct EidLayout {
+  uint32_t* keys;
+  uint32_t* keys_alt;
+  uint32_t* vals;
+  uint32_t* vals_alt;
+  void* sort_tmp;
+  size_t sort_bytes;
+  size_t total;
+};
+
+EidLayout eid_layout(void* ws, int64_t E, int64_t n_dst) {
+  Carve c(ws, ~size_t(0));
+  EidLayout L;
+  L.keys = c.take<uint32_t>(E);
+  L.keys_alt = c.take<uint32_t>(E);
+  L.vals = c.take<uint32_t>(E);
+  L.vals_alt = c.take<uint32_t>(E);
+  L.sort_bytes = 0;
+  rocprim::double_buffer<uint32_t> k(nullptr, nullptr), v(nullptr, nullptr);
+  (void)rocprim::radix_sort_pairs(nullptr, L.sort_bytes, k, v, (unsigned)E, 0, csr_end_bit(n_dst), 0, false);
   L.sort_tmp = c.take<char>(L.sort_bytes);
   L.total = c.used();
   return L;
@@ -450,19 +616,13 @@
 
 using namespace kgx;
 
-extern "C" int kgx_csr_workspace_bytes(int64_t E, int64_t n_dst, int flags, size_t* bytes) {
-  KGX_REQUIRE(bytes && E >= 0 && n_dst >= 0, KGX_ERR_ARG, "kgx_csr_workspace_bytes: bad arguments");
-  const int64_t total = E + ((flags & KGX_CSR_SELF_LOOPS) ? n_dst : 0);
-  *bytes = csr_layout(nullptr, total, n_dst).total;
-  return KGX_OK;
-}
-
-extern "C" int kgx_csr_build2(const int32_t* src, const int32_t* dst, int64_t E, int64_t n_src,
-                              int64_t n_dst, int flags, int32_t* rowptr, int32_t* col, int32_t* eid,
-                              int32_t* deg, float* dinv, float* w, const float* dinv_table,
-                              int64_t table_len, void* workspace, size_t workspace_bytes, int64_t* info,
-                              kgx_stream_t stream_) {
-  hipStream_t stream = as_stream(stream_);
+namespace kgx {
+namespace {
+
+int csr_enqueue(const int32_t* src, const int32_t* dst, int64_t E, int64_t n_src, int64_t n_dst, int flags,
+                int32_t* rowptr, int32_t* col, int32_t* eid, int32_t* deg, float* dinv, float* w,
+                const float* dinv_table, int64_t table_len, void* workspace, size_t workspace_bytes,
+                CsrStatus* st, CsrStatus** st_out, hipStream_t stream) {
   const bool loops = flags & KGX_CSR_SELF_LOOPS;
   const bool norm = flags & KGX_CSR_GCN_NORM;
   KGX_REQUIRE(E >= 0 && n_dst >= 0 && n_src >= 0, KGX_ERR_ARG, "kgx_csr_build: negative sizes");
@@ -472,31 +632,73 @@
   const int64_t total = E + (loops ? n_dst : 0);
   KGX_REQUIRE(total < (int64_t(1) << 31) - 1 && n_dst < (int64_t(1) << 31) - 1, KGX_ERR_ARG,
               "kgx_csr_build: graph too large for int32 CSR (E'=%lld)", (long long)total);
-  KGX_REQUIRE(rowptr && deg && (total == 0 || (col && eid)), KGX_ERR_ARG, "kgx_csr_build: null output");
+  KGX_REQUIRE(rowptr && deg && (total == 0 || col), KGX_ERR_ARG, "kgx_csr_build: null output");
   KGX_REQUIRE(E == 0 || (src && dst), KGX_ERR_ARG, "kgx_csr_build: null input");
   KGX_REQUIRE(!norm || (dinv && (total == 0 || w)), KGX_ERR_ARG, "kgx_csr_build: GCN_NORM needs dinv and w");
   KGX_REQUIRE(!dinv_table || table_len > 0, KGX_ERR_ARG, "kgx_csr_build2: empty dinv table");
+  const int end_bit = csr_end_bit(n_dst);
+
+  if (!eid) {
+    Csr64Layout L = csr64_layout(workspace, E, n_dst);
+    KGX_REQUIRE(workspace && workspace_bytes >= L.total, KGX_ERR_ARG,
+                "kgx_csr_build: workspace %zu < %zu bytes", workspace_bytes, L.total);
+    if (!st) {
+      st = L.st;
+      KGX_CHECK_HIP(hipMemsetAsync(st, 0, sizeof(CsrStatus), stream));
+    }
+    const uint64_t* sorted = L.keys;
+    if (E > 0) {
+      hipLaunchKernelGGL(csr_prep64_kernel, dim3(grid_for(E, 8192)), dim3(kBlock), 0, stream, src, dst, E, n_src,
+                         n_dst, flags, L.keys, st);
+      KGX_CHECK_LAUNCH();
+      rocprim::double_buffer<uint64_t> keys(L.keys, L.keys_alt);
+      size_t sb = L.sort_bytes;
+      KGX_CHECK_HIP(rocprim::radix_sort_keys(L.sort_tmp, sb, keys, (unsigned)E, 32, 32 + end_bit, stream, false));
+      sorted = keys.current();
+    }
+    hipLaunchKernelGGL((csr_rowptr_kernel<uint64_t, 32>), dim3(grid_for(n_dst + 1, 8192)), dim3(kBlock), 0, stream,
+                       sorted, E, n_dst, loops ? 1 : 0, rowptr, st);
+    KGX_CHECK_LAUNCH();
+    if (n_dst > 0) {
+      hipLaunchKernelGGL(csr_deg_kernel, dim3(grid_for(n_dst, 1024)), dim3(kBlock), 0, stream, rowptr, n_dst, flags,
+                         deg, dinv, dinv_table, table_len, st, loops ? col : nullptr, loops ? w : nullptr);
+      KGX_CHECK_LAUNCH();
+    }
+    if (E > 0) {
+      const dim3 grid(grid_for(E / kColIlp + 1, 8192));
+      if (norm)
+        hipLaunchKernelGGL(csr_col64_kernel<true>, grid, dim3(kBlock), 0, stream, sorted, rowptr, n_dst,
+                           loops ? 1 : 0, dinv, col, w);
+      else
+        hipLaunchKernelGGL(csr_col64_kernel<false>, grid, dim3(kBlock), 0, stream, sorted, rowptr, n_dst,
+                           loops ? 1 : 0, dinv, col, w);
+      KGX_CHECK_LAUNCH();
+    }
+    if (st_out) *st_out = st;
+    return KGX_OK;
+  }
+
   CsrLayout L = csr_layout(workspace, total, n_dst);
   KGX_REQUIRE(workspace && workspace_bytes >= L.total, KGX_ERR_ARG,
               "kgx_csr_build: workspace %zu < %zu bytes", workspace_bytes, L.total);
-
-  KGX_CHECK_HIP(hipMemsetAsync(L.st, 0, sizeof(CsrStatus), stream));
+  if (!st) {
+    st = L.st;
+    KGX_CHECK_HIP(hipMemsetAsync(st, 0, sizeof(CsrStatus), stream));
+  }
   if (total > 0) {
     hipLaunchKernelGGL(csr_prep_kernel, dim3(grid_for(total, 8192)), dim3(kBlock), 0, stream, src, dst, E,
-                       n_src, n_dst, flags, L.keys, L.vals, L.st);
+                       n_src, n_dst, flags, L.keys, L.vals, st);
     KGX_CHECK_LAUNCH();
-    const int end_bit = ceil_log2_u64(uint64_t(n_dst) + 1);
     size_t sb = L.sort_bytes;
     KGX_CHECK_HIP(rocprim::radix_sort_pairs(L.sort_tmp, sb, L.keys, L.keys_sorted, L.vals, L.vals_sorted,
-                                            (unsigned)total, 0, end_bit > 0 ? end_bit : 1, stream,
-                                            false));
-  }
-  hipLaunchKernelGGL(csr_rowptr_kernel, dim3(grid_for(n_dst + 1, 8192)), dim3(kBlock), 0, stream,
-                     L.keys_sorted, total, n_dst, rowptr, L.st);
+                                            (unsigned)total, 0, end_bit, stream, false));
+  }
+  hipLaunchKernelGGL((csr_rowptr_kernel<uint32_t, 0>), dim3(grid_for(n_dst + 1, 8192)), dim3(kBlock), 0, stream,
+                     L.keys_sorted, total, n_dst, 0, rowptr, st);
   KGX_CHECK_LAUNCH();
   if (n_dst > 0) {
     hipLaunchKernelGGL(csr_deg_kernel, dim3(grid_for(n_dst, 1024)), dim3(kBlock), 0, stream, rowptr, n_dst,
-                       flags, deg, dinv, dinv_table, table_len, L.st);
+                       flags, deg, dinv, dinv_table, table_len, st, (int32_t*)nullptr, (float*)nullptr);
     KGX_CHECK_LAUNCH();
   }
   if (total > 0) {
@@ -509,9 +711,74 @@
                          n_dst, dinv, eid, col, w);
     KGX_CHECK_LAUNCH();
   }
+  if (st_out) *st_out = st;
+  return KGX_OK;
+}
+
+int sched_enqueue(const int32_t* rowptr, int64_t n_dst, int32_t split_len, int32_t* rows, int32_t* items,
+                  int64_t cap_items, int32_t* split, void* workspace, size_t workspace_bytes, SchedStatus* st,
+                  SchedStatus** st_out, hipStream_t stream) {
+  KGX_REQUIRE(rowptr && n_dst > 0, KGX_ERR_ARG, "kgx_schedule_build: bad arguments");
+  KGX_REQUIRE(split_len <= 0 || (split_len & (split_len - 1)) == 0, KGX_ERR_ARG,
+              "kgx_schedule_build: split_len must be a power of two (got %d)", split_len);
+  KGX_REQUIRE(rows && items && split, KGX_ERR_ARG, "kgx_schedule_build: null output");
+  SchedLayout L = sched_layout(workspace, n_dst);
+  KGX_REQUIRE(workspace && workspace_bytes >= L.total, KGX_ERR_ARG,
+              "kgx_schedule_build: workspace %zu < %zu bytes", workspace_bytes, L.total);
+  if (!st) {
+    st = L.st;
+    KGX_CHECK_HIP(hipMemsetAsync(st, 0, sizeof(SchedStatus), stream));
+  }
+  const unsigned g = grid_for(n_dst, 8192);
+  hipLaunchKernelGGL(sched_keys_kernel, dim3(g), dim3(kBlock), 0, stream, rowptr, n_dst, L.keys, L.iota);
+  KGX_CHECK_LAUNCH();
+  size_t tb = L.tmp_bytes;
+  KGX_CHECK_HIP(rocprim::radix_sort_pairs(L.tmp, tb, L.keys, L.keys_sorted, L.iota, rows, (unsigned)n_dst, 0,
+                                          kDegKeyBits, stream, false));
+  hipLaunchKernelGGL(sched_count_kernel, dim3(g), dim3(kBlock), 0, stream, rowptr, rows, n_dst, split_len,
+                     L.nchunks, L.nslots);
+  KGX_CHECK_LAUNCH();
+  tb = L.tmp_bytes;
+  KGX_CHECK_HIP(rocprim::exclusive_scan(L.tmp, tb, (const int32_t*)L.nchunks, L.item_off, 0, (size_t)n_dst,
+                                        rocprim::plus<int32_t>(), stream, false));
+  tb = L.tmp_bytes;
+  KGX_CHECK_HIP(rocprim::exclusive_scan(L.tmp, tb, (const int32_t*)L.nslots, L.slot_off, 0, (size_t)n_dst,
+                                        rocprim::plus<int32_t>(), stream, false));
+  hipLaunchKernelGGL(sched_emit_kernel, dim3(g), dim3(kBlock), 0, stream, rowptr, rows, n_dst, split_len,
+                     L.nchunks, L.item_off, L.nslots, L.slot_off, reinterpret_cast<int4*>(items), cap_items,
+                     reinterpret_cast<int4*>(split), st);
+  KGX_CHECK_LAUNCH();
+  if (st_out) *st_out = st;
+  return KGX_OK;
+}
+
+}
+}
+
+extern "C" int kgx_csr_workspace_bytes2(int64_t E, int64_t n_dst, int flags, int with_eid, size_t* bytes) {
+  KGX_REQUIRE(bytes && E >= 0 && n_dst >= 0, KGX_ERR_ARG, "kgx_csr_workspace_bytes: bad arguments");
+  const int64_t total = E + ((flags & KGX_CSR_SELF_LOOPS) ? n_dst : 0);
+  *bytes = with_eid ? csr_layout(nullptr, total, n_dst).total : csr64_layout(nullptr, E, n_dst).total;
+  return KGX_OK;
+}
+
+extern "C" int kgx_csr_workspace_bytes(int64_t E, int64_t n_dst, int flags, size_t* bytes) {
+  return kgx_csr_workspace_bytes2(E, n_dst, flags, 1, bytes);
+}
+
+extern "C" int kgx_csr_build2(const int32_t* src, const int32_t* dst, int64_t E, int64_t n_src,
+                              int64_t n_dst, int flags, int32_t* rowptr, int32_t* col, int32_t* eid,
+                              int32_t* deg, float* dinv, float* w, const float* dinv_table,
+                              int64_t table_len, void* workspace, size_t workspace_bytes, int64_t* info,
+                              kgx_stream_t stream_) {
+  hipStream_t stream = as_stream(stream_);
+  CsrStatus* st = nullptr;
+  const int rc = csr_enqueue(src, dst, E, n_src, n_dst, flags, rowptr, col, eid, deg, dinv, w, dinv_table, table_len,
+                             workspace, workspace_bytes, nullptr, &st, stream);
+  if (rc != KGX_OK) return rc;
   CsrStatus hs;
-  KGX_CHECK_HIP(hipMemcpyAsync(&hs, L.st, sizeof(CsrStatus), hipMemcpyDeviceToHost, stream));
-  KGX_CHECK_HIP(hipStreamSynchronize(stream));
+  KGX_CHECK_HIP(hipMemcpyAsync(&hs, st, sizeof(CsrStatus), hipMemcpyDeviceToHost, stream));
+  KGX_CHECK_HIP(sync_counted(stream));
   if (info) {
     info[0] = int64_t(hs.kept);
     info[1] = int64_t(hs.max_deg);
@@ -532,6 +799,44 @@
   return kgx_csr_build2(src, dst, E, n_src, n_dst, flags, rowptr, col, eid, deg, dinv, w, nullptr, 0, workspace,
                         workspace_bytes, info, stream_);
 }
+
+extern "C" int kgx_csr_eid_workspace_bytes(int64_t E, int64_t n_dst, size_t* bytes) {
+  KGX_REQUIRE(bytes && E >= 0 && n_dst >= 0, KGX_ERR_ARG, "kgx_csr_eid_workspace_bytes: bad arguments");
+  *bytes = eid_layout(nullptr, E, n_dst).total;
+  return KGX_OK;
+}
+
+extern "C" int kgx_csr_eid(const int32_t* dst, int64_t E, int64_t n_dst, int flags, const int32_t* rowptr,
+                           int32_t* eid, void* workspace, size_t workspace_bytes, kgx_stream_t stream_) {
+  hipStream_t stream = as_stream(stream_);
+  const bool loops = flags & KGX_CSR_SELF_LOOPS;
+  KGX_REQUIRE(E >= 0 && n_dst >= 0 && rowptr, KGX_ERR_ARG, "kgx_csr_eid: bad arguments");
+  const int64_t total = E + (loops ? n_dst : 0);
+  KGX_REQUIRE(total < (int64_t(1) << 31) - 1, KGX_ERR_ARG, "kgx_csr_eid: graph too large for int32 CSR");
+  if (total == 0) return KGX_OK;
+  KGX_REQUIRE(eid && (E == 0 || dst), KGX_ERR_ARG, "kgx_csr_eid: null pointer");
+  EidLayout L = eid_layout(workspace, E, n_dst);
+  KGX_REQUIRE(workspace && workspace_bytes >= L.total, KGX_ERR_ARG, "kgx_csr_eid: workspace %zu < %zu bytes",
+              workspace_bytes, L.total);
+  const uint32_t *ks = L.keys, *vs = L.vals;
+  if (E > 0) {
+    hipLaunchKernelGGL(eid_prep_kernel, dim3(grid_for(E, 8192)), dim3(kBlock), 0, stream, dst, E, n_dst, L.keys,
+                       L.vals);
+    KGX_CHECK_LAUNCH();
+    rocprim::double_buffer<uint32_t> keys(L.keys, L.keys_alt), vals(L.vals, L.vals_alt);
+    size_t sb = L.sort_bytes;
+    KGX_CHECK_HIP(rocprim::radix_sort_pairs(L.sort_tmp, sb, keys, vals, (unsigned)E, 0, csr_end_bit(n_dst), stream,
+                                            false));
+    ks = keys.current();
+    vs = vals.current();
+  }
+  hipLaunchKernelGGL(eid_place_kernel, dim3(grid_for(E > n_dst ? E : n_dst, 8192)), dim3(kBlock), 0, stream, ks, vs,
+                     rowptr, E, n_dst, loops ? 1 : 0, eid);
+  KGX_CHECK_LAUNCH();
+  return KGX_OK;
+}
+
+extern "C" int64_t kgx_graph_sync_count(void) { return int64_t(g_stream_syncs.load(std::memory_order_relaxed)); }
 
 extern "C" int kgx_schedule_workspace_bytes(int64_t n_dst, size_t* bytes) {
   KGX_REQUIRE(bytes && n_dst >= 0, KGX_ERR_ARG, "kgx_schedule_workspace_bytes: bad arguments");
@@ -550,33 +855,13 @@
     if (info) info[0] = info[1] = info[2] = info[3] = 0;
     return KGX_OK;
   }
-  KGX_REQUIRE(rows && items && split, KGX_ERR_ARG, "kgx_schedule_build: null output");
-  SchedLayout L = sched_layout(workspace, n_dst);
-  KGX_REQUIRE(workspace && workspace_bytes >= L.total, KGX_ERR_ARG,
-              "kgx_schedule_build: workspace %zu < %zu bytes", workspace_bytes, L.total);
-  KGX_CHECK_HIP(hipMemsetAsync(L.st, 0, sizeof(SchedStatus), stream));
-  const unsigned g = grid_for(n_dst, 8192);
-  hipLaunchKernelGGL(sched_keys_kernel, dim3(g), dim3(kBlock), 0, stream, rowptr, n_dst, L.keys, L.iota);
-  KGX_CHECK_LAUNCH();
-  size_t tb = L.tmp_bytes;
-  KGX_CHECK_HIP(rocprim::radix_sort_pairs(L.tmp, tb, L.keys, L.keys_sorted, L.iota, rows, (unsigned)n_dst, 0,
-                                          kDegKeyBits, stream, false));
-  hipLaunchKernelGGL(sched_count_kernel, dim3(g), dim3(kBlock), 0, stream, rowptr, rows, n_dst, split_len,
-                     L.nchunks, L.nslots);
-  KGX_CHECK_LAUNCH();
-  tb = L.tmp_bytes;
-  KGX_CHECK_HIP(rocprim::exclusive_scan(L.tmp, tb, (const int32_t*)L.nchunks, L.item_off, 0, (size_t)n_dst,
-                                        rocprim::plus<int32_t>(), stream, false));
-  tb = L.tmp_bytes;
-  KGX_CHECK_HIP(rocprim::exclusive_scan(L.tmp, tb, (const int32_t*)L.nslots, L.slot_off, 0, (size_t)n_dst,
-                                        rocprim::plus<int32_t>(), stream, false));
-  hipLaunchKernelGGL(sched_emit_kernel, dim3(g), dim3(kBlock), 0, stream, rowptr, rows, n_dst, split_len,
-                     L.nchunks, L.item_off, L.nslots, L.slot_off, reinterpret_cast<int4*>(items), cap_items,
-                     reinterpret_cast<int4*>(split), L.st);
-  KGX_CHECK_LAUNCH();
+  SchedStatus* st = nullptr;
+  const int rc = sched_enqueue(rowptr, n_dst, split_len, rows, items, cap_items, split, workspace, workspace_bytes,
+                               nullptr, &st, stream);
+  if (rc != KGX_OK) return rc;
   SchedStatus hs;
-  KGX_CHECK_HIP(hipMemcpyAsync(&hs, L.st, sizeof(SchedStatus), hipMemcpyDeviceToHost, stream));
-  KGX_CHECK_HIP(hipStreamSynchronize(stream));
+  KGX_CHECK_HIP(hipMemcpyAsync(&hs, st, sizeof(SchedStatus), hipMemcpyDeviceToHost, stream));
+  KGX_CHECK_HIP(sync_counted(stream));
   KGX_REQUIRE(hs.overflow == 0, KGX_ERR_ARG, "kgx_schedule_build: cap_items %lld too small",
               (long long)cap_items);
   if (info) {
@@ -655,7 +940,7 @@
   KGX_CHECK_LAUNCH();
   unsigned long long h = 0;
   KGX_CHECK_HIP(hipMemcpyAsync(&h, cnt, sizeof(h), hipMemcpyDeviceToHost, stream));
-  KGX_CHECK_HIP(hipStreamSynchronize(stream));
+  KGX_CHECK_HIP(sync_counted(stream));
   *n_out = int64_t(h);
   return KGX_OK;
 }
@@ -763,7 +1048,7 @@
   hipLaunchKernelGGL(cu_census_kernel, dim3(unsigned(n_blocks)), dim3(64), 0, cs->tail, tail_ids, n_blocks);
   KGX_CHECK_LAUNCH();
   KGX_CHECK_HIP(sj.join());
-  KGX_CHECK_HIP(hipStreamSynchronize(s));
+  KGX_CHECK_HIP(sync_counted(s));
   n_cus[0] = cs->n_head;
   n_cus[1] = cs->n_tail;
   return KGX_OK;
@@ -772,8 +1057,19 @@
 namespace kgx {
 namespace {
 
+struct BuildStatus {
+  CsrStatus csr;
+  SchedStatus sched;
+  unsigned long long suffix[2];
+  unsigned long long tiny[2];
+  unsigned long long tiny_start;
+  unsigned long long tiny_n;
+};
+
 __global__ void sched_suffix_kernel(const int4* __restrict__ items, int64_t n, int short_max, int tiny_max,
-                                    unsigned long long* __restrict__ out) {
+                                    unsigned long long* __restrict__ out,
+                                    const unsigned long long* __restrict__ n_dev) {
+  if (n_dev) n = int64_t(*n_dev) < n ? int64_t(*n_dev) : n;
   const int64_t stride = int64_t(gridDim.x) * blockDim.x;
   unsigned long long ls = 0, lt = 0;
   for (int64_t i = int64_t(blockIdx.x) * blockDim.x + threadIdx.x; i < n; i += stride) {
@@ -806,7 +1102,23 @@
 
 __global__ void tiny_pack_kernel(const int4* __restrict__ items, int64_t start, int64_t n,
                                  const int32_t* __restrict__ col, const float* __restrict__ w, int64_t n_col,
-                                 int4* __restrict__ pack, float2* __restrict__ tw, unsigned long long* __restrict__ st) {
+                                 int4* __restrict__ pack, float2* __restrict__ tw, unsigned long long* __restrict__ st,
+                                 BuildStatus* __restrict__ bs, int short_on, int64_t min_rows) {
+  if (bs) {
+    const int64_t n_items = int64_t(bs->sched.n_items);
+    const int64_t n_long = short_on ? int64_t(bs->suffix[0]) : n_items;
+    int64_t s0 = int64_t(bs->suffix[1]);
+    if (n_long >= 0 && n_long <= n_items && n_long > s0) s0 = n_long;
+    int64_t m = n_items - s0;
+    n_col = int64_t(bs->csr.kept);
+    if (m < min_rows || m > n || n_col <= 0) m = 0;
+    start = s0;
+    n = m;
+    if (blockIdx.x == 0 && threadIdx.x == 0) {
+      bs->tiny_start = (unsigned long long)s0;
+      bs->tiny_n = (unsigned long long)m;
+    }
+  }
   const int64_t stride = int64_t(gridDim.x) * blockDim.x;
   unsigned long long cnt = 0, last2 = 0;
   for (int64_t i = int64_t(blockIdx.x) * blockDim.x + threadIdx.x; i < n; i += stride) {
@@ -858,12 +1170,12 @@
   KGX_CHECK_HIP(hipMemsetAsync(st, 0, 2 * sizeof(unsigned long long), s));
   if (n_items > 0) {
     hipLaunchKernelGGL(sched_suffix_kernel, dim3(grid_for(n_items, 1024)), dim3(kBlock), 0, s,
-                       reinterpret_cast<const int4*>(items), n_items, short_max, tiny_max, st);
+                       reinterpret_cast<const int4*>(items), n_items, short_max, tiny_max, st, nullptr);
     KGX_CHECK_LAUNCH();
   }
   unsigned long long h[2];
   KGX_CHECK_HIP(hipMemcpyAsync(h, st, sizeof(h), hipMemcpyDeviceToHost, s));
-  KGX_CHECK_HIP(hipStreamSynchronize(s));
+  KGX_CHECK_HIP(sync_counted(s));
   out[0] = int64_t(h[0]);
   out[1] = int64_t(h[1]);
   return KGX_OK;
@@ -880,13 +1192,109 @@
   if (n > 0) {
     hipLaunchKernelGGL(tiny_pack_kernel, dim3(grid_for(n, 2048)), dim3(kBlock), 0, s,
                        reinterpret_cast<const int4*>(items), start, n, col, tw ? w : nullptr, n_col,
-                       reinterpret_cast<int4*>(pack), reinterpret_cast<float2*>(tw), st);
+                       reinterpret_cast<int4*>(pack), reinterpret_cast<float2*>(tw), st, nullptr, 0, 0);
     KGX_CHECK_LAUNCH();
   }
   unsigned long long h[2];
   KGX_CHECK_HIP(hipMemcpyAsync(h, st, sizeof(h), hipMemcpyDeviceToHost, s));
-  KGX_CHECK_HIP(hipStreamSynchronize(s));
+  KGX_CHECK_HIP(sync_counted(s));
   out[0] = int64_t(h[0]);
   out[1] = int64_t(h[1]);
   return KGX_OK;
 }
+
+namespace kgx {
+namespace {
+
+BuildStatus* pinned_status() {
+  thread_local BuildStatus* p = nullptr;
+  if (!p && hipHostMalloc(reinterpret_cast<void**>(&p), sizeof(BuildStatus), hipHostMallocPortable) != hipSuccess)
+    p = nullptr;
+  return p;
+}
+
+struct BuildLayout {
+  BuildStatus* bs;
+  void* stage;
+  size_t stage_bytes;
+  size_t total;
+};
+
+BuildLayout build_layout(void* ws, int64_t E, int64_t n_dst) {
+  Carve c(ws, ~size_t(0));
+  BuildLayout L;
+  L.bs = c.take<BuildStatus>(1);
+  const size_t a = csr64_layout(nullptr, E, n_dst).total;
+  const size_t b = n_dst > 0 ? sched_layout(nullptr, n_dst).total : 0;
+  L.stage_bytes = a > b ? a : b;
+  L.stage = c.take<char>(L.stage_bytes);
+  L.total = c.used();
+  return L;
+}
+
+}
+}
+
+extern "C" int kgx_graph_build_workspace_bytes(int64_t E, int64_t n_dst, int flags, size_t* bytes) {
+  (void)flags;
+  KGX_REQUIRE(bytes && E >= 0 && n_dst >= 0, KGX_ERR_ARG, "kgx_graph_build_workspace_bytes: bad arguments");
+  *bytes = build_layout(nullptr, E, n_dst).total;
+  return KGX_OK;
+}
+
+extern "C" int kgx_graph_build(const int32_t* src, const int32_t* dst, int64_t E, int64_t n_src, int64_t n_dst,
+                               int flags, int32_t* rowptr, int32_t* col, int32_t* deg, float* dinv, float* w,
+                               const float* dinv_table, int64_t table_len, int32_t split_len, int32_t* rows,
+                               int32_t* items, int64_t cap_items, int32_t* split, int short_max, int tiny_max,
+                               int64_t tiny_min_rows, int32_t* pack, float* tw, int64_t tiny_cap, void* workspace,
+                               size_t workspace_bytes, int64_t* info, kgx_stream_t stream_) {
+  hipStream_t stream = as_stream(stream_);
+  KGX_REQUIRE(info && E >= 0 && n_dst >= 0, KGX_ERR_ARG, "kgx_graph_build: bad arguments");
+  KGX_REQUIRE(!pack || tiny_cap > 0, KGX_ERR_ARG, "kgx_graph_build: tiny records without capacity");
+  BuildLayout L = build_layout(workspace, E, n_dst);
+  KGX_REQUIRE(workspace && workspace_bytes >= L.total, KGX_ERR_ARG, "kgx_graph_build: workspace %zu < %zu bytes",
+              workspace_bytes, L.total);
+  BuildStatus* host = pinned_status();
+  KGX_REQUIRE(host != nullptr, KGX_ERR_HIP, "kgx_graph_build: no pinned host block");
+  KGX_CHECK_HIP(hipMemsetAsync(L.bs, 0, sizeof(BuildStatus), stream));
+  int rc = csr_enqueue(src, dst, E, n_src, n_dst, flags, rowptr, col, nullptr, deg, dinv, w, dinv_table, table_len,
+                       L.stage, L.stage_bytes, &L.bs->csr, nullptr, stream);
+  if (rc != KGX_OK) return rc;
+  if (n_dst > 0) {
+    rc = sched_enqueue(rowptr, n_dst, split_len, rows, items, cap_items, split, L.stage, L.stage_bytes,
+                       &L.bs->sched, nullptr, stream);
+    if (rc != KGX_OK) return rc;
+    hipLaunchKernelGGL(sched_suffix_kernel, dim3(grid_for(cap_items, 1024)), dim3(kBlock), 0, stream,
+                       reinterpret_cast<const int4*>(items), cap_items, short_max < 0 ? 0 : short_max, tiny_max,
+                       L.bs->suffix, &L.bs->sched.n_items);
+    KGX_CHECK_LAUNCH();
+    if (pack && col) {
+      hipLaunchKernelGGL(tiny_pack_kernel, dim3(grid_for(tiny_cap, 2048)), dim3(kBlock), 0, stream,
+                         reinterpret_cast<const int4*>(items), int64_t(0), tiny_cap, col, tw ? w : nullptr,
+                         int64_t(0), reinterpret_cast<int4*>(pack), reinterpret_cast<float2*>(tw), L.bs->tiny, L.bs,
+                         short_max < 0 ? 0 : 1, tiny_min_rows);
+      KGX_CHECK_LAUNCH();
+    }
+  }
+  KGX_CHECK_HIP(hipMemcpyAsync(host, L.bs, sizeof(BuildStatus), hipMemcpyDeviceToHost, stream));
+  KGX_CHECK_HIP(sync_counted(stream));
+  const BuildStatus hs = *host;
+  info[0] = int64_t(hs.csr.kept);
+  info[1] = int64_t(hs.csr.max_deg);
+  info[2] = int64_t(hs.csr.bad);
+  info[3] = int64_t(hs.csr.table_miss);
+  info[4] = int64_t(hs.sched.n_items);
+  info[5] = int64_t(hs.sched.n_split);
+  info[6] = int64_t(hs.sched.n_slots);
+  info[7] = short_max < 0 ? int64_t(hs.sched.n_items) : int64_t(hs.suffix[0]);
+  info[8] = int64_t(hs.tiny_start);
+  info[9] = int64_t(hs.tiny_n);
+  info[10] = int64_t(hs.tiny[0]);
+  info[11] = int64_t(hs.tiny[1]);
+  KGX_REQUIRE(hs.csr.bad == 0, KGX_ERR_INDEX,
+              "index out of range in edge_index: %llu edge(s) reference a node outside "
+              "[-n, n) (n_src=%lld, n_dst=%lld)",
+              hs.csr.bad, (long long)n_src, (long long)n_dst);
+  KGX_REQUIRE(hs.sched.overflow == 0, KGX_ERR_ARG, "kgx_graph_build: cap_items %lld too small", (long long)cap_items);
+  return KGX_OK;
+}
diff --git a/keras-geometric_amd/keras_geometric_amd/_native.py b/keras-geometric_amd/keras_geometric_amd/_native.py
--- a/keras-geometric_amd/keras_geometric_amd/_native.py
+++ b/keras-geometric_amd/keras_geometric_amd/_native.py
@@ -41,6 +41,16 @@
         _i32p, _i32p, _i32p, _i32p, _f32p, _f32p, _f32p, _i64,
         ctypes.c_void_p, ctypes.c_size_t, ctypes.POINTER(ctypes.c_int64), ctypes.c_void_p,
     ],
+    "kgx_csr_workspace_bytes2": [_i64, _i64, _int, _int, ctypes.POINTER(ctypes.c_size_t)],
+    "kgx_csr_eid_workspace_bytes": [_i64, _i64, ctypes.POINTER(ctypes.c_size_t)],
+    "kgx_csr_eid": [_i32p, _i64, _i64, _int, _i32p, _i32p, ctypes.c_void_p, ctypes.c_size_t, ctypes.c_void_p],
+    "kgx_graph_build_workspace_bytes": [_i64, _i64, _int, ctypes.POINTER(ctypes.c_size_t)],
+    "kgx_graph_build": [
+        _i32p, _i32p, _i64, _i64, _i64, _int, _i32p, _i32p, _i32p, _f32p, _f32p, _f32p, _i64,
+        ctypes.c_int32, _i32p, _i32p, _i64, _i32p, _int, _int, _i64, _i32p, _f32p, _i64,
+        ctypes.c_void_p, ctypes.c_size_t, ctypes.POINTER(ctypes.c_int64), ctypes.c_void_p,
+    ],
+    "kgx_graph_sync_count": [],
     "kgx_gcn_dinv": [_i32p, _i64, _f32p, ctypes.c_void_p],
     "kgx_cu_split_layout_ok": [_int, _int, ctypes.c_char_p],
     "kgx_schedule_suffixes": [_i32p, _i64, _int, _int, ctypes.c_void_p, ctypes.POINTER(ctypes.c_int64),
@@ -154,7 +164,7 @@
         ctypes.c_void_p, ctypes.c_size_t, ctypes.POINTER(ctypes.c_int64), ctypes.c_void_p,
     ],
 }
-_RESTYPES = {"kgx_last_error": ctypes.c_char_p}
+_RESTYPES = {"kgx_last_error": ctypes.c_char_p, "kgx_graph_sync_count": ctypes.c_int64}
 
 _lib: ctypes.CDLL | None = None
 
diff --git a/keras-geometric_amd/keras_geometric_amd/graph.py b/keras-geometric_amd/keras_geometric_amd/graph.py
--- a/keras-geometric_amd/keras_geometric_amd/graph.py
+++ b/keras-geometric_amd/keras_geometric_amd/graph.py
@@ -28,6 +28,42 @@
 
 def exact_mode_default() -> bool:
     return os.environ.get("KGX_EXACT", "0") not in ("", "0", "false", "False")
+
+
+class _LazyEid:
+
+    __slots__ = ("dst", "version", "E", "n_dst", "flags", "rowptr", "kept", "stream", "value")
+
+    def __init__(self, dst, E, n_dst, flags, rowptr, kept, stream):
+        self.dst, self.version, self.E, self.n_dst, self.flags = dst, dst._version, E, n_dst, flags
+        self.rowptr, self.kept, self.stream, self.value = rowptr, kept, stream, None
+
+    def get(self) -> torch.Tensor:
+        if self.value is not None:
+            return self.value
+        if self.dst._version != self.version:
+            raise RuntimeError("CSRGraph.eid: the edge_index this graph was built from was modified in place "
+                               "before its edge ids were first read; rebuild the graph")
+        dev = self.rowptr.device
+        L = nat.lib()
+        cap = self.E + (self.n_dst if self.flags & nat.CSR_SELF_LOOPS else 0)
+        nbytes = ctypes.c_size_t(0)
+        nat.check(L.kgx_csr_eid_workspace_bytes(self.E, self.n_dst, ctypes.byref(nbytes)),
+                  "kgx_csr_eid_workspace_bytes")
+        with torch.cuda.stream(self.stream):
+            eid = torch.empty(max(cap, 1), dtype=torch.int32, device=dev)
+            ws = torch.empty(max(nbytes.value, 1), dtype=torch.uint8, device=dev)
+            nat.check(L.kgx_csr_eid(nat.ptr(self.dst), self.E, self.n_dst, self.flags, nat.ptr(self.rowptr),
+                                    nat.ptr(eid), nat.ptr(ws), nbytes.value,
+                                    ctypes.c_void_p(self.stream.cuda_stream)), "kgx_csr_eid")
+            del ws
+        cur = torch.cuda.current_stream(dev)
+        if cur != self.stream:
+            cur.wait_stream(self.stream)
+            eid.record_stream(cur)
+        self.value = eid[: self.kept]
+        self.dst = None
+        return self.value
 
 
 @dataclass
@@ -58,10 +94,25 @@
     def device(self) -> torch.device:
         return self.rowptr.device
 
+    def _get_eid(self):
+        v = self.__dict__.get("_eid")
+        return v.get() if isinstance(v, _LazyEid) else v
+
+    def _set_eid(self, v) -> None:
+        self.__dict__["_eid"] = v
+
+    @property
+    def eid_ready(self) -> bool:
+        v = self.__dict__.get("_eid")
+        return not (isinstance(v, _LazyEid) and v.value is None)
+
     def work(self, exact: bool):
         if exact or self.n_items == 0:
             return None, 0, None, 0, 0
         return self.items, self.n_items, self.split, self.n_split, self.n_slots
+
+
+CSRGraph.eid = property(CSRGraph._get_eid, CSRGraph._set_eid)
 
 
 _DINV_TABLES: dict = {}
@@ -118,29 +169,50 @@
     )
     cap = E + (n_dst if self_loops else 0)
     L = nat.lib()
+    from . import tiny
+
     i32 = dict(dtype=torch.int32, device=dev)
+    f32 = dict(dtype=torch.float32, device=dev)
     rowptr = torch.empty(n_dst + 1, **i32)
     col = torch.empty(max(cap, 1), **i32)
-    eid = torch.empty(max(cap, 1), **i32)
     deg = torch.empty(max(n_dst, 1), **i32)
-    dinv = torch.empty(max(n_dst, 1), dtype=torch.float32, device=dev) if gcn_norm else None
-    w = torch.empty(max(cap, 1), dtype=torch.float32, device=dev) if gcn_norm else None
+    dinv = torch.empty(max(n_dst, 1), **f32) if gcn_norm else None
+    w = torch.empty(max(cap, 1), **f32) if gcn_norm else None
+    spec_split = split_len if split_len is not None else default_split_len(cap, n_features)
+    if spec_split > 0:
+        spec_split = _pow2_floor(spec_split)
+    chunks = cap // spec_split if spec_split > 0 else 0
+    cap_items = n_dst + chunks + 1
+    cap_split = min(n_dst, chunks + 1)
+    rows = torch.empty(n_dst, **i32)
+    items = torch.empty((cap_items, 4), **i32)
+    split = torch.empty((max(cap_split, 1), 4), **i32)
+    short_on = os.environ.get("KGX_SHORT_ROWS", "1") not in ("0", "false", "False")
+    short_max = int(os.environ.get("KGX_SHORT_MAX", SHORT_ROW_MAX)) if short_on else -1
+    tiny_on = n_dst > 0 and os.environ.get("KGX_TINY", "1") not in ("0", "false", "False")
+    pack = torch.empty((n_dst, 4), **i32) if tiny_on else None
+    tw = torch.empty((n_dst, 2), **f32) if tiny_on and gcn_norm else None
     nbytes = ctypes.c_size_t(0)
-    nat.check(L.kgx_csr_workspace_bytes(E, n_dst, flags, ctypes.byref(nbytes)), "kgx_csr_workspace_bytes")
+    nat.check(L.kgx_graph_build_workspace_bytes(E, n_dst, flags, ctypes.byref(nbytes)),
+              "kgx_graph_build_workspace_bytes")
     ws = torch.empty(max(nbytes.value, 1), dtype=torch.uint8, device=dev)
-    info = (ctypes.c_int64 * 4)()
+    info = (ctypes.c_int64 * 12)()
     table = gcn_dinv_table(dev) if gcn_norm else None
+    stream = torch.cuda.current_stream(dev)
     nat.check(
-        L.kgx_csr_build2(
+        L.kgx_graph_build(
             nat.ptr(src), nat.ptr(dst), E, n_src, n_dst, flags,
-            nat.ptr(rowptr), nat.ptr(col), nat.ptr(eid), nat.ptr(deg), nat.ptr(dinv), nat.ptr(w),
+            nat.ptr(rowptr), nat.ptr(col), nat.ptr(deg), nat.ptr(dinv), nat.ptr(w),
             nat.ptr(table), table.numel() if table is not None else 0,
-            nat.ptr(ws), nbytes.value, info, nat.stream(dev),
+            spec_split, nat.ptr(rows), nat.ptr(items), cap_items, nat.ptr(split),
+            short_max, tiny.TINY_MAX, tiny._MIN_ROWS, nat.ptr(pack), nat.ptr(tw), n_dst,
+            nat.ptr(ws), nbytes.value, info, ctypes.c_void_p(stream.cuda_stream),
         ),
-        "kgx_csr_build2",
+        "kgx_graph_build",
     )
     del ws
     kept, max_deg = int(info[0]), int(info[1])
+    redo_tiny = False
     if gcn_norm and int(info[3]):
         table = gcn_dinv_table(dev, max_deg)
         st = nat.stream(dev)
@@ -148,12 +220,38 @@
                   "kgx_gcn_dinv_table")
         nat.check(L.kgx_gcn_edge_norm(nat.ptr(rowptr), nat.ptr(col), n_dst, nat.ptr(dinv), nat.ptr(dinv),
                                       nat.ptr(w), st), "kgx_gcn_edge_norm")
+        redo_tiny = True
     g = CSRGraph(
         n_src=n_src, n_dst=n_dst, n_input_edges=E, kept=kept, max_degree=max_deg, flags=flags,
-        rowptr=rowptr, col=col[:kept], eid=eid[:kept], deg=deg[:n_dst],
+        rowptr=rowptr, col=col[:kept], eid=_LazyEid(dst, E, n_dst, flags, rowptr, kept, stream), deg=deg[:n_dst],
         dinv=dinv[:n_dst] if dinv is not None else None, w=w[:kept] if w is not None else None,
     )
-    _build_schedule(g, split_len if split_len is not None else default_split_len(kept, n_features))
+    want_split = split_len if split_len is not None else default_split_len(kept, n_features)
+    if want_split > 0:
+        want_split = _pow2_floor(want_split)
+    if want_split != spec_split:
+        _build_schedule(g, want_split)
+        return g
+    g.split_len = spec_split
+    g.rows = rows
+    if n_dst == 0:
+        return g
+    g.n_items, g.n_split, g.n_slots = int(info[4]), int(info[5]), int(info[6])
+    if g.n_split > cap_split:
+        raise RuntimeError("kgx schedule: split list overflow")
+    g.items = items[: g.n_items]
+    g.split = split[: max(g.n_split, 0)]
+    g.n_long = int(info[7])
+    if redo_tiny:
+        _refresh_tiny(g)
+        return g
+    t_start, t_n, n2, last2 = int(info[8]), int(info[9]), int(info[10]), int(info[11])
+    res = (None, None, -1, 0)
+    if tiny_on and t_n > 0:
+        if n2 and last2 != n2:
+            n2 = t_n
+        res = (pack[:t_n], tw[:t_n] if tw is not None else None, t_start, n2)
+    g._kgx_tiny, g._kgx_tiny_w = res, g.w
     return g
 
 
@@ -362,12 +460,13 @@
 def restrict_rows(g: CSRGraph, row_mask: torch.Tensor) -> CSRGraph:
     from dataclasses import replace
 
+    lazy = g.__dict__.get("_eid")
     if g.n_items == 0:
-        return replace(g, extras={})
+        return replace(g, eid=lazy, extras={})
     keep = row_mask[g.items[:, 0].long()]
     items = g.items[keep].contiguous()
     split = g.split[row_mask[g.split[:, 0].long()]].contiguous() if g.n_split else g.split
-    sub = replace(g, items=items, split=split, n_items=int(items.shape[0]), n_split=int(split.shape[0]) if g.n_split
+    sub = replace(g, eid=lazy, items=items, split=split, n_items=int(items.shape[0]), n_split=int(split.shape[0]) if g.n_split
                   else 0, extras={"restricted_of": g})
     sub.n_long = short_suffix_start(items)
     _refresh_tiny(sub)
```

Result: no change. 12.79 billion edges/s (-0.4%).
